# 2gunsu/monocon-pytorch

Measured on AMD Instinct MI355X. Metric: images/sec (384x1280) fwd+bwd, higher is better.
Workload: dtype f32 (f16x2); 1 GPU; train step B=32/GPU 3x384x1280 (configs[2] shape, fp32 values, mode f16x2); global_batch=32, parallelism=dp1, precision_mode=f16x2

## Files before the change

### include/monocon_hip.h

```cpp
#ifndef MONOCON_HIP_H
#define MONOCON_HIP_H

#include <stddef.h>
#include <stdint.h>

#ifdef __cplusplus
extern "C" {
#endif

typedef struct mc_handle mc_handle;

enum { MC_F32 = 0, MC_I64 = 1 };

typedef struct mc_tensor_desc {
    const char *name;
    void *ptr;
    int64_t numel;
    int32_t dtype;
} mc_tensor_desc;

enum {
    MC_PRED_CENTER_HEATMAP = 0, MC_PRED_KPT_HEATMAP, MC_PRED_WH, MC_PRED_OFFSET,
    MC_PRED_KPT_HEATMAP_OFFSET, MC_PRED_CENTER2KPT_OFFSET, MC_PRED_DIM, MC_PRED_DEPTH,
    MC_PRED_ALPHA_CLS, MC_PRED_ALPHA_OFFSET, MC_NUM_PREDS
// ... 32 lines not shown
        *alpha_offset_target, *depth_target, *center2kpt_offset_target, *kpt_heatmap_target,
        *kpt_heatmap_offset_target;
    int64_t *indices, *indices_kpt;
    uint8_t *mask_target;
    float *mask_center2kpt_offset, *mask_kpt_heatmap_offset;
} mc_targets;
int mc_make_targets(mc_handle *h, const mc_labels *labels, int B, int max_objs, int pad_h,
                    int pad_w, int feat_h, int feat_w, const mc_targets *targets, void *stream);
int mc_losses(mc_handle *h, const float *const preds[MC_NUM_PREDS], const mc_targets *targets,
              int B, int max_objs, int feat_h, int feat_w, float *losses, void *stream);
int mc_losses_backward(mc_handle *h, const float *const preds[MC_NUM_PREDS],
                       const mc_targets *targets, int B, int max_objs, int feat_h, int feat_w,
                       const float *grad_losses, float *const dpreds[MC_NUM_PREDS], void *stream);
int mc_losses_backward_pred(mc_handle *h, const float *const preds[MC_NUM_PREDS],
                            const mc_targets *targets, int B, int max_objs, int feat_h, int feat_w,
                            const float *grad_losses, float *const dpreds[MC_NUM_PREDS], void *stream);

int mc_forward_train(mc_handle *h, const float *img, const mc_labels *labels, int B, int H, int W,
                     int max_objs, float *const preds[MC_NUM_PREDS], float *losses, void *stream);
int mc_backward(mc_handle *h, const float *grad_losses, void *stream);
int mc_backward_pred_grads(mc_handle *h, const float *grad_losses, const float *const grad_preds[MC_NUM_PREDS],
                           void *stream);
int mc_backward_image_grad(mc_handle *h, const float *grad_losses, const float *const grad_preds[MC_NUM_PREDS],
                           float *grad_img, void *stream);
int mc_train_generation(mc_handle *h, unsigned long long *generation);
int mc_head_forward_train(mc_handle *h, const float *feat, const mc_labels *labels, int B, int pad_h, int pad_w,
                          int max_objs, float *const preds[MC_NUM_PREDS], float *losses, void *stream);
int mc_head_backward(mc_handle *h, const float *grad_losses, float *grad_feat, void *stream);
int mc_head_backward_pred_grads(mc_handle *h, const float *grad_losses, const float *const grad_preds[MC_NUM_PREDS],
                                float *grad_feat, void *stream);
int mc_train_debug_node(mc_handle *h, int node, int which, float *out_nchw, int dims[4], void *stream);
int mc_infer_debug_node(mc_handle *h, int node, int which, float *out_nchw, int dims[4], void *stream);

int mc_comm_unique_id(mc_handle *h, void *id128);
int mc_comm_init(mc_handle *h, int rank, int world, const void *id128);
int mc_comm_destroy(mc_handle *h);
int mc_comm_set_overlap(mc_handle *h, int on);
int mc_comm_info(mc_handle *h, int *rank, int *world, int *overlap, int *n_collectives, unsigned long long *launches,
                 char *lib_path, int lib_path_len);
int mc_comm_exposed_ms(mc_handle *h, float *ms);
int mc_allreduce_grads(mc_handle *h, void *stream);
int mc_build_train_plan(mc_handle *h, int B, int H, int W);
int mc_tune_export(mc_handle *h, int *buf, int cap, int *n_ints);
int mc_tune_import(mc_handle *h, const int *buf, int n_ints);

int mc_optim_bind(mc_handle *h, int n, float *const params[], float *const grads[],
                  float *const exp_avg[], float *const exp_avg_sq[], const int64_t numel[]);
int mc_clip_adamw_step(mc_handle *h, double lr, double beta1, double beta2, double eps,
                       double weight_decay, double max_norm, int step, float *out_norm, void *stream);

#define MC_OPT_MAX_CLASSES 16
typedef struct mc_optim_class {
    double lr, beta1, beta2, eps, weight_decay;
    int step, amsgrad, maximize;
} mc_optim_class;
int mc_optim_bind_classes(mc_handle *h, int n, float *const params[], float *const grads[],
                          float *const exp_avg[], float *const exp_avg_sq[],
                          float *const max_exp_avg_sq[], const int64_t numel[], const int cls[]);
int mc_clip_adamw_step_classes(mc_handle *h, const mc_optim_class *classes, int ncls, double max_norm,
                               double norm_type, float *out_norm, void *stream);
int mc_clip_bind(mc_handle *h, int n, float *const grads[], const int64_t numel[]);
int mc_clip_grad_norm(mc_handle *h, double max_norm, double norm_type, float *out_norm, void *stream);

int mc_op_conv(mc_handle *h, const float *const src[], const int src_channels[], int nsrc,
               int B, int Hin, int Win, const float *weight_oihw, int Cout, int ksize,
               int stride, const float *scale, const float *bias, const float *residual,
               int relu, float *out, void *stream);
int mc_op_conv_wgrad(mc_handle *h, const float *const src[], const int src_channels[], int nsrc,
                     int B, int Hin, int Win, const float *dy, int Cout, int ksize, int stride,
                     float *dw_oihw, void *stream);
int mc_op_stem(mc_handle *h, const float *img_nchw, int B, int H, int W,
               const float *weight_oihw, const float *scale, const float *bias, float *out,
               void *stream);
int mc_op_stem_dgrad(mc_handle *h, const float *dy_nhwc, const float *weight_oihw, int B, int H, int W,
                     float *dx_nchw, void *stream);
int mc_op_stem_dgrad_fused(mc_handle *h, const float *d_nhwc, const float *y_nhwc, const float *coef,
                           const float *weight_oihw, int B, int H, int W, float *dx_nchw, void *stream);
int mc_op_maxpool2(mc_handle *h, const float *in, int B, int H, int W, int C, float *out,
                   void *stream);
int mc_op_deconv4x4(mc_handle *h, const float *in, int B, int H, int W, int C,
                    const float *weight, float *out, void *stream);
int mc_op_conv_dgrad(mc_handle *h, const float *dy, const float *weight_oihw, int B, int Hin, int Win, int CinTotal,
                     int c_off, int Cs, int Cout, int ksize, int stride, int accumulate, float *dx, void *stream);
int mc_op_nchw_to_nhwc(mc_handle *h, const float *in, int B, int C, int H, int W, float *out,
                       void *stream);
int mc_op_nhwc_to_nchw(mc_handle *h, const float *in, int B, int C, int H, int W, float *out,
                       void *stream);

int mc_preprocess(mc_handle *h, const void *img_hwc, int dtype, int H, int W, const double mean[3],
                  const double std[3], int pad_h, int pad_w, float *out_chw, void *stream);

int mc_preprocess_augmented(mc_handle *h, const unsigned char *frames_hwc, const float *params, int B, int src_h, int src_w,
                            const double mean[3], const double std[3], int pad_h, int pad_w, float *out_bchw, void *stream);

int mc_kitti_format(mc_handle *h, const float *box2d, const float *box3d, const int64_t *cls, const uint8_t *keep_thr,
                    const float *P2, const float *img_hw_scale, int B, int K, float *rows3d, int *n3d, float *rows2d,
                    int *n2d, void *stream);

int mc_nms3d(mc_handle *h, const float *box2d, const float *box3d, const int64_t *cls, const uint8_t *keep_in,
             int B, int K, int mode, float iou_thr, int class_agnostic,
             uint8_t *keep_out, int *suppressed_by, void *stream);

int mc_rotate_iou_eval(mc_handle *h, const float *boxes, const float *query_boxes, long long N, long long K,
                       int criterion, float *iou, void *stream);
int mc_box3d_overlap(mc_handle *h, const double *boxes, const double *query_boxes, long long N, long long K,
                     int criterion, double *overlap, void *stream);

int mc_kitti_image_overlap(const double *boxes, long long N, const double *query_boxes, long long K, int criterion,
                           double *overlap);
int mc_kitti_statistics_part(int mode, const double *overlaps, long long n_frames, const long long *gt_nums,
                             const long long *dt_nums, const long long *dc_nums, const double *gt_datas,
                             const double *dt_datas, const double *dontcares, const long long *ignored_gts,
                             const long long *ignored_dets, int metric, double min_overlap, const double *thresholds,
                             long long n_thresholds, int compute_aos, double *pr, double *scores_out,
                             long long *n_scores);

int mc_query_workspace(mc_handle *h, int B, int H, int W, int mode, size_t *bytes);

int mc_profile_train(mc_handle *h, int iters, double ms[3], double flops[3], double bytes[3], int launches[3],
                     void *stream);
int mc_set_precision(mc_handle *h, int mode);
int mc_set_conv_cfg(mc_handle *h, int cfg);
int mc_bench_conv(mc_handle *h, int B, int Hin, int Win, int nsrc, const int src_channels[],
                  int Cout, int ksize, int stride, int cfg, int iters, float *ms_avg);

int mc_bench_mfma_peak(mc_handle *h, int waves_per_simd, int iters, float *tflops);

size_t mc_workspace_bytes(mc_handle *h);
int mc_forward_cost(mc_handle *h, int B, int H, int W, double flops[2], double bytes[2]);
int mc_profile_forward(mc_handle *h, int iters, float out_ms[3], int out_n[3], void *stream);

#ifdef __cplusplus
}
#endif
#endif
```

### monocon-pytorch_amd/csrc/conv_bf16.hip

```cpp
#include "conv_mfma.h"

namespace mc {

typedef __bf16 bf16x8 __attribute__((ext_vector_type(8)));
typedef __bf16 bf16x4 __attribute__((ext_vector_type(4)));
typedef _Float16 f16x8 __attribute__((ext_vector_type(8)));
typedef _Float16 f16x4 __attribute__((ext_vector_type(4)));

template <int SPL> struct Piece { typedef __bf16 T; typedef bf16x8 V8; typedef bf16x4 V4; };
template <> struct Piece<2> { typedef _Float16 T; typedef f16x8 V8; typedef f16x4 V4; };
__device__ __forceinline__ f32x16 mfma_k16(bf16x8 a, bf16x8 b, f32x16 c) { return __builtin_amdgcn_mfma_f32_32x32x16_bf16(a, b, c, 0, 0, 0); }
__device__ __forceinline__ f32x16 mfma_k16(f16x8 a, f16x8 b, f32x16 c) { return __builtin_amdgcn_mfma_f32_32x32x16_f16(a, b, c, 0, 0, 0); }

template <int KS, int S, int WM, int WN, int WTM, int WTN, int SPL>
struct ConvCfgB16 {
    static constexpr int CK = 32;
    static constexpr int PB = WM * WTM, BNT = WN * WTN * 32, NT = 64 * WM * WN;
    static constexpr int KH = win_h(KS), KW = win_w(KS), PAD = win_pad(KS);
    static constexpr int IH = 3 * S + KH, IW = 7 * S + KW, NPIX = IH * IW;
    static constexpr int ROWB = (CK + 8) * 2;
    static constexpr bool PLANAR = S == 1;
    static constexpr int RS = 24;
    static constexpr int PPB = IH * RS * 16;
    static constexpr int CPL = ((PB + 1) / 2) * PPB + 32;
    static_assert(!PLANAR || (2 * IW <= RS && CK == 32), "two patches per 24-slot row, four 16-byte chunks per pixel");
    static constexpr int PLANE_BYTES = PLANAR ? 4 * CPL : PB * NPIX * ROWB;
    static constexpr int TILE_BYTES = SPL * PLANE_BYTES;
    static constexpr size_t LDS_BYTES = TILE_BYTES + PB * 16;
};

template <int KS, int S, int WM, int WN, int WTM, int WTN, int SPL, bool BM = false, bool LZ = false>
__global__ __launch_bounds__(64 * WM * WN, SPL == 1 ? 3 : 2) void conv_bf16_kernel(const ConvArgs a) {
    static_assert(!LZ || (SPL == 2 && !BM), "lazy sources: forward launches of the fp16-split mode");
    using Cfg = ConvCfgB16<KS, S, WM, WN, WTM, WTN, SPL>;
    typedef typename Piece<SPL>::T pc_t;
    typedef typename Piece<SPL>::V8 pc8;
    typedef typename Piece<SPL>::V4 pc4;
    constexpr int PLANE = Cfg::PLANE_BYTES;
    constexpr int CK = Cfg::CK, PB = Cfg::PB, BNT = Cfg::BNT, NT = Cfg::NT, PAD = Cfg::PAD;
    constexpr int IW = Cfg::IW, NPIX = Cfg::NPIX, ROWB = Cfg::ROWB;
    constexpr bool PLANAR = Cfg::PLANAR;
    constexpr int RS = Cfg::RS, PPB = Cfg::PPB, CPL = Cfg::CPL;
    constexpr int C4 = CK / 4;
    static_assert(NT % C4 == 0, "a thread keeps one channel group across its staging elements");

    extern __shared__ __attribute__((aligned(16))) unsigned char lds_raw[];
    int *pinfo = reinterpret_cast<int *>(lds_raw + Cfg::TILE_BYTES);

    const int tid = threadIdx.x;
    const int lane = tid & 63;
    const int wave = __builtin_amdgcn_readfirstlane(tid >> 6);
    const int wm = wave / WN, wn = wave % WN;
    const int g = lane >> 5, li = lane & 31;

    int img, chunk, n0;
    conv_wg<BNT>(a, img, chunk, n0);

    unsigned am_raw[4] = {0u, 0u, 0u, 0u};
    if constexpr (SPL == 2) {
        const int al = lane < AMAX_SUB ? lane * AMAX_STRIDE : 0;
#pragma unroll
        for (int i = 0; i < 4; ++i) am_raw[i] = a.amax_in[i < a.nsrc ? i : 0][al];
    }

    if (tid < PB) {
        const int pp = chunk * PB + tid;
        const int valid = pp < a.ppi;
        const int py = pp / a.ppr, px = pp % a.ppr;
        pinfo[tid * 4 + 0] = img;
        pinfo[tid * 4 + 1] = py * 4;
        pinfo[tid * 4 + 2] = px * 8;
        pinfo[tid * 4 + 3] = valid;
    }
    __syncthreads();

    float a_scale = 1.f, omul = 1.f;
    auto operand_scales = [&] {
        if constexpr (SPL == 2) {
            unsigned v = am_raw[0];
#pragma unroll
            for (int i = 1; i < 4; ++i) v = am_raw[i] > v ? am_raw[i] : v;
            v = lane < AMAX_SUB ? v : 0u;
#pragma unroll
            for (int o = 8; o > 0; o >>= 1) { const unsigned t = (unsigned)__shfl_xor((int)v, o); v = t > v ? t : v; }
            const int ea = f16_scale_exp((unsigned)__builtin_amdgcn_readfirstlane((int)v));
            const int ew = f16_scale_exp(*a.amax_w);
            a_scale = exp2i(ea);
            omul = exp2i(-ea) * exp2i(-ew);
        }
    };
    constexpr int NACC = SPL >= 2 ? 2 : 1;
    f32x16 acc[WTM][WTN], accm[NACC == 2 ? WTM : 1][NACC == 2 ? WTN : 1];
#pragma unroll
    for (int tm = 0; tm < WTM; ++tm)
#pragma unroll
        for (int tn = 0; tn < WTN; ++tn)
#pragma unroll
            for (int r = 0; r < 16; ++r) {
                acc[tm][tn][r] = 0.f;
                if (NACC == 2) accm[tm][tn][r] = 0.f;
            }

    constexpr int TOTAL = PB * NPIX * C4;
    constexpr int NIT = (TOTAL + NT - 1) / NT;
    const int c4 = tid % C4;
    unsigned char *stage_dst = lds_raw + (tid / C4) * ROWB + c4 * 8;

    int a_off[WTM];
#pragma unroll
    for (int tm = 0; tm < WTM; ++tm) {
        const int p = wm * WTM + tm;
        a_off[tm] = PLANAR ? g * CPL + (p >> 1) * PPB + ((li >> 3) * RS + (li & 7) + IW * (p & 1)) * 16
                           : (p * NPIX + ((li >> 3) * S) * IW + (li & 7) * S) * ROWB + g * 16;
    }

    const int Cin8 = a.Cin >> 3;
    const int w_plane = Cfg::KH * Cfg::KW * a.Cin * a.CoutP * 2;
    const __amdgpu_buffer_rsrc_t r_w = make_rsrc(a.wpk16, (unsigned)(SPL * w_plane));
    const int w_lane = (g * a.CoutP + n0 + wn * WTN * 32 + li) * 16;

    constexpr int KSTEPS = CK / 16, NS = Cfg::KH * Cfg::KW * KSTEPS;
    auto load_b = [&](pc8(&dst)[SPL][WTN], int kc, int s) {
        const int tap = s / KSTEPS, m = s % KSTEPS;
        const int soff = (tap * Cin8 + ((kc + m * 16) >> 3)) * a.CoutP * 16;
#pragma unroll
        for (int q = 0; q < SPL; ++q)
#pragma unroll
            for (int tn = 0; tn < WTN; ++tn)
                dst[q][tn] = __builtin_bit_cast(
                    pc8, __builtin_amdgcn_raw_buffer_load_b128(r_w, w_lane + tn * 32 * 16, soff + q * w_plane, 0));
    };
    auto load_a = [&](pc8(&dst)[SPL][WTM], int s) {
        const int tap = s / KSTEPS, m = s % KSTEPS;
#pragma unroll
        for (int q = 0; q < SPL; ++q)
#pragma unroll
            for (int tm = 0; tm < WTM; ++tm)
                dst[q][tm] = *reinterpret_cast<const pc8 *>(
                    lds_raw + q * PLANE + a_off[tm] +
                    (PLANAR ? 2 * m * CPL + ((tap / Cfg::KW) * RS + (tap % Cfg::KW)) * 16
                            : ((tap / Cfg::KW) * IW + (tap % Cfg::KW)) * ROWB + m * 32));
    };
#ifndef MC_CONV_DB_REGS
#define MC_CONV_DB_REGS 48
#endif
    constexpr int DB_FIT = MC_CONV_DB_REGS / (SPL * WTN * 4);
    constexpr int DB = (WTM * WTN > 2) ? 2 : ((DB_FIT >= 6 && NS % 6 == 0) ? 6 : ((DB_FIT >= 3 && NS % 3 == 0) ? 3 : 2));
    static_assert(NS % DB == 0, "ring slots must line up across K-chunks");
    pc8 bq[DB][SPL][WTN];
#pragma unroll
    for (int j = 0; j < DB - 1; ++j) load_b(bq[j], 0, j);
    const EpiCoef<WTN> coef = conv_epi_coef<WN, WTN, BM>(a, n0, wn, li);

#ifndef MC_CONV_PF
#define MC_CONV_PF 1
#endif
    constexpr bool PF = MC_CONV_PF && NIT <= 8 && WTM * WTN <= 2;
    constexpr int UB = NIT > 8 ? 8 : NIT;
    f32x4 pv[PF ? NIT : 1];
    int voff[NIT], sdst[NIT];
    int si = 0, c0 = 0, kc = 0;
    int Cs = a.src[0].C;
    f32x4 lzA = {0.f, 0.f, 0.f, 0.f}, lzB = lzA;
    bool lz_cur = false, lz_next = false;
    auto lazy_fetch = [&](int s_idx, int cc0) {
        if constexpr (LZ) {
            lz_next = a.src[s_idx].la != nullptr;
            if (lz_next) {
                lzA = reinterpret_cast<const f32x4 *>(a.src[s_idx].la + cc0)[c4];
                lzB = reinterpret_cast<const f32x4 *>(a.src[s_idx].lb + cc0)[c4];
            }
        }
    };
    auto lazy_advance = [&] {
        if constexpr (LZ) {
            lz_cur = lz_next;
            if (lz_cur) {
#pragma unroll
                for (int j = 0; j < 4; ++j) { lzA[j] *= a_scale; lzB[j] *= a_scale; }
            }
        }
    };
    __amdgpu_buffer_rsrc_t r_in = make_rsrc(a.src[0].p + (size_t)img * a.Hin * a.Win * Cs, (unsigned)(a.Hin * a.Win * Cs) * 4u);
    auto lane_offsets = [&](int cs) {
#pragma unroll
        for (int i = 0; i < NIT; ++i) {
            const int e = tid + NT * i;
            const int t = e / C4;
            const int pix = t % NPIX;
            const int p = (t / NPIX) % PB;
            const int iy = pix / IW, ix = pix % IW;
            const int y = pinfo[p * 4 + 1] * S - PAD + iy;
            const int x = pinfo[p * 4 + 2] * S - PAD + ix;
            const bool ok = (e < TOTAL) & (pinfo[p * 4 + 3] != 0) & ((unsigned)y < (unsigned)a.Hin) & ((unsigned)x < (unsigned)a.Win);
            int off = ((y * a.Win + x) * cs + c4 * 4) * 4;
            asm volatile("" : "+v"(off));
            voff[i] = ok ? off : BUF_OOB;
            sdst[i] = PLANAR ? (c4 >> 1) * CPL + (p >> 1) * PPB + (iy * RS + ix + IW * (p & 1)) * 16 + (c4 & 1) * 8
                             : (int)(stage_dst - lds_raw) + i * (NT / C4) * ROWB;
        }
    };
    auto stage_load = [&](__amdgpu_buffer_rsrc_t r, int vo, int so) -> f32x4 { return buf_load4(r, vo, so); };
    auto stage_one = [&](const f32x4 &v, int i, auto lz_c) {
        constexpr bool LZC = decltype(lz_c)::value;
        if (i < NIT && (NT * (i + 1) <= TOTAL || tid + NT * i < TOTAL)) {
            pc4 q[SPL];
            [[maybe_unused]] const float cap = voff[i] != BUF_OOB ? __builtin_inff() : 0.f;
#pragma unroll
            for (int j = 0; j < 4; ++j) {
                float r = SPL == 2 ? (LZC ? lazy_act(v[j], lzA[j], lzB[j], cap) : v[j] * a_scale) : v[j];
#pragma unroll
                for (int pz = 0; pz < SPL; ++pz) {
                    q[pz][j] = (pc_t)r;
                    r -= (float)q[pz][j];
                }
            }
#pragma unroll
            for (int pz = 0; pz < SPL; ++pz) *reinterpret_cast<pc4 *>(lds_raw + sdst[i] + pz * PLANE) = q[pz];
        }
    };
#ifdef MC_PHASE_TIMERS
    unsigned long long tp_stage = 0, tp_bar = 0, tp_mfma = 0, tp_epi = 0;
    const unsigned long long tp_t0 = __builtin_readcyclecounter();
#define TP_NOW() __builtin_readcyclecounter()
#else
#define TP_NOW() 0ull
#endif
    lane_offsets(Cs);
    lazy_fetch(0, 0);
    if (PF) {
#pragma unroll
        for (int i = 0; i < NIT; ++i) pv[i] = stage_load(r_in, voff[i], 0);
    }
    __builtin_amdgcn_sched_barrier(0);
    operand_scales();
// ... 12 lines not shown
                    f32x4 v[UB];
#pragma unroll
                    for (int u = 0; u < UB; ++u)
                        if (i0 + u < NIT) v[u] = stage_load(r_in, voff[i0 + u], c0 * 4);
#pragma unroll
                    for (int u = 0; u < UB; ++u) stage_one(v[u], i0 + u, lz_c);
                }
            }
        };
        if constexpr (LZ) {
            if (lz_cur) stage_chunk(std::true_type{});
            else stage_chunk(std::false_type{});
        } else {
            stage_chunk(std::false_type{});
        }
        [[maybe_unused]] unsigned long long tp_c = TP_NOW();
        __syncthreads();
        [[maybe_unused]] unsigned long long tp_d = TP_NOW();
        int nsi = si, nc0 = c0 + CK;
        if (nc0 >= Cs) { ++nsi; nc0 = 0; }
        const bool more = nsi < a.nsrc;
        if (more && nsi != si) {
            Cs = a.src[nsi].C;
            r_in = make_rsrc(a.src[nsi].p + (size_t)img * a.Hin * a.Win * Cs, (unsigned)(a.Hin * a.Win * Cs) * 4u);
            lane_offsets(Cs);
        }
        if (more) lazy_fetch(nsi, nc0);
        if (PF && more) {
#pragma unroll
            for (int i = 0; i < NIT; ++i) pv[i] = stage_load(r_in, voff[i], nc0 * 4);
        }
        {
            const int kc_next = (kc + CK < a.Cin) ? kc + CK : kc;
            pc8 acur[SPL][WTM];
            load_a(acur, 0);
#pragma unroll
            for (int s = 0; s < NS; ++s) {
                pc8 anext[SPL][WTM];
                if (s + 1 < NS) load_a(anext, s + 1);
                {
                    const int t = s + DB - 1;
                    if (t < NS) load_b(bq[t % DB], kc, t);
                    else load_b(bq[t % DB], kc_next, t - NS);
                }
                __builtin_amdgcn_sched_barrier(0);
                constexpr int NP = SPL == 1 ? 1 : (SPL == 2 ? 3 : 6);
                constexpr int PA[6] = {SPL == 2 ? 1 : 0, SPL == 2 ? 0 : 2, SPL == 2 ? 0 : 1, 0, 1, 0};
                constexpr int PBv[6] = {SPL == 2 ? 0 : 2, SPL == 2 ? 1 : 0, SPL == 2 ? 0 : 1, 1, 0, 0};
#pragma unroll
                for (int pp = 0; pp < NP; ++pp)
#pragma unroll
                    for (int tm = 0; tm < WTM; ++tm)
#pragma unroll
                        for (int tn = 0; tn < WTN; ++tn) {
                            if (NACC == 2 && pp < NP - 1)
                                accm[tm][tn] = mfma_k16(acur[PA[pp]][tm], bq[s % DB][PBv[pp]][tn], accm[tm][tn]);
                            else
                                acc[tm][tn] = mfma_k16(acur[SPL == 1 ? 0 : PA[pp]][tm], bq[s % DB][SPL == 1 ? 0 : PBv[pp]][tn], acc[tm][tn]);
                        }
                if (s + 1 < NS) {
#pragma unroll
                    for (int q = 0; q < SPL; ++q)
#pragma unroll
                        for (int tm = 0; tm < WTM; ++tm) acur[q][tm] = anext[q][tm];
                }
            }
        }
#ifdef MC_PHASE_TIMERS
        { const unsigned long long tp_e = TP_NOW(); tp_bar += (tp_b - tp_a) + (tp_d - tp_c); tp_stage += tp_c - tp_b; tp_mfma += tp_e - tp_d; }
#endif
        if (!more) break;
        si = nsi; c0 = nc0; kc += CK;
    }
    [[maybe_unused]] const unsigned long long tp_f = TP_NOW();

    if (NACC == 2) {
#pragma unroll
        for (int tm = 0; tm < WTM; ++tm)
#pragma unroll
            for (int tn = 0; tn < WTN; ++tn)
#pragma unroll
                for (int r = 0; r < 16; ++r) acc[tm][tn][r] += accm[tm][tn][r];
    }
    conv_epilogue<WM, WN, WTM, WTN, BNT, BM>(a, acc, pinfo, chunk * PB, img, n0, wm, wn, g, li, coef, omul);
#ifdef MC_PHASE_TIMERS
    if (a.phase_prof && lane == 0) {
        __builtin_amdgcn_s_waitcnt(0);
        const unsigned long long tp_g = TP_NOW();
        tp_epi = tp_g - tp_f;
        unsigned long long *o = a.phase_prof + ((size_t)blockIdx.x * (NT / 64) + wave) * 5;
        o[0] = tp_stage; o[1] = tp_bar; o[2] = tp_mfma; o[3] = tp_epi; o[4] = tp_g - tp_t0;
    }
#endif
}

template <int KS, int S, class Sh, int SPL, bool BM = false, bool LZ = false>
static hipError_t launch_b16_one(ConvArgs a, hipStream_t st, ConvArgs *resolved) {
    using Cfg = ConvCfgB16<KS, S, Sh::WM, Sh::WN, Sh::WTM, Sh::WTN, SPL>;
    static_assert(Cfg::PB == Sh::PB && Cfg::BNT == Sh::BNT, "the shape table and the kernel agree on the tile");
    if constexpr (!LZ) {
        if (conv_any_lazy(a)) {
            if constexpr (SPL == 2 && !BM && (KS == 3 || KS == 1)) {
                if (a.bm_y) return hipErrorInvalidValue;
                return launch_b16_one<KS, S, Sh, SPL, false, true>(a, st, resolved);
            } else {
                return hipErrorInvalidValue;
            }
        }
    }
    if constexpr (!BM && S == 1 && (KS == 3 || KS == 1)) {
        if (a.bm_y) return launch_b16_one<KS, S, Sh, SPL, true>(a, st, resolved);
    } else if constexpr (!BM) {
        if (a.bm_y) return hipErrorInvalidValue;
    }
    conv_set_patches(a, Cfg::PB);
    if (a.CoutP % Cfg::BNT) return hipErrorInvalidValue;
    if (resolved) *resolved = a;
    return launch_dyn_lds<conv_bf16_kernel<KS, S, Sh::WM, Sh::WN, Sh::WTM, Sh::WTN, SPL, BM, LZ>>(
        Cfg::LDS_BYTES, dim3((unsigned)(a.B * a.chunks * (a.CoutP / Cfg::BNT))), dim3(Cfg::NT), st, a);
}

bool conv_bf16_ok(const ConvArgs &a, int ks, int stride) {
    if (!a.wpk16) return false;
    if (a.prec == 3) {
        if (!a.amax_w) return false;
        for (int i = 0; i < a.nsrc; ++i)
            if (!a.amax_in[i]) return false;
    }
    for (int i = 0; i < a.nsrc; ++i)
        if (a.src[i].C % 32) return false;
    if (ks == 3) return stride == 1 || stride == 2;
    return stride == 1 && (ks == 1 || ks == 12 || ks == 21 || ks == 22);
}

template <int SPL>
static hipError_t launch_conv_b16_spl(const ConvArgs &a, int ks, int stride, hipStream_t st, ConvArgs *resolved) {
    return with_conv_window(ks, stride, [&](auto win) {
        return with_conv_shape(a.cfg, [&](auto sh) {
            return launch_b16_one<decltype(win)::KS, decltype(win)::S, decltype(sh), SPL>(a, st, resolved);
        });
    });
}

hipError_t launch_conv_bf16(const ConvArgs &a, int ks, int stride, hipStream_t st, ConvArgs *resolved) {
    if (!conv_bf16_ok(a, ks, stride)) return hipErrorInvalidValue;
    if (a.prec == 3) return launch_conv_b16_spl<2>(a, ks, stride, st, resolved);
    return a.prec == 2 ? launch_conv_b16_spl<3>(a, ks, stride, st, resolved) : launch_conv_b16_spl<1>(a, ks, stride, st, resolved);
}

}
```

### monocon-pytorch_amd/csrc/conv_mfma.h

```cpp
#pragma once
#include <hip/hip_runtime.h>
#include <stdint.h>
#include <atomic>
#include <type_traits>
#include <utility>

namespace mc {

typedef float f32x16 __attribute__((ext_vector_type(16)));
typedef float f32x4 __attribute__((ext_vector_type(4)));

struct DynLdsOnce {
    std::atomic<unsigned long long> done{0};
    hipError_t ensure(const void *fn, int bytes) {
        int dev = 0;
        if (hipGetDevice(&dev) != hipSuccess || dev < 0 || dev >= 64) return hipFuncSetAttribute(fn, hipFuncAttributeMaxDynamicSharedMemorySize, bytes);
        if ((done.load(std::memory_order_acquire) >> dev) & 1ull) return hipSuccess;
        const hipError_t e = hipFuncSetAttribute(fn, hipFuncAttributeMaxDynamicSharedMemorySize, bytes);
        if (e == hipSuccess) done.fetch_or(1ull << dev, std::memory_order_release);
        return e;
    }
};

struct ConvSrc {
    const float *p;
    int C;
    const float *la, *lb;
};
__device__ __forceinline__ float lazy_act(float y, float a, float b, float cap) {
    return __builtin_amdgcn_fmed3f(__builtin_fmaf(y, a, b), 0.f, cap);
}

struct ConvArgs {
    ConvSrc src[4];
    int nsrc;
    int B, Hin, Win, Hout, Wout;
    int Cin;
    int Cout, CoutP;
    const float *wpk;
    const float *scale;
    const float *bias;
    const float *res;
    int res_ld;
    float *out;
    int out_ld, out_coff;
    int relu;
    float *stats;
    const float *stat_shift;
    int stats_centred;
    int ppr, ppi, chunks;
    int cfg;
    int o_img, o_row, o_px, r_img, r_row, r_px;
    const void *wpk16;
    int prec;
    const float *bm_y;
    const float *bm_z;
    const unsigned *bm_zbits;
    const float *bm_a, *bm_b;
    int bm_relu;
    const unsigned *amax_in[4];
    const unsigned *amax_w;
    unsigned *amax_out;
    unsigned long long *phase_prof;
};

__host__ __device__ __forceinline__ int f16_scale_exp(unsigned amax_bits) {
    const int E = (int)((amax_bits >> 23) & 0xffu);
    if (E == 0) return 0;
    const int e = 141 - E;
    return e > 126 ? 126 : e;
}
__host__ __device__ __forceinline__ float exp2i(int e) {
    const unsigned u = (unsigned)(127 + e) << 23;
    return __builtin_bit_cast(float, u);
}
constexpr int AMAX_SUB = 16, AMAX_STRIDE = 64, AMAX_WORDS = AMAX_SUB * AMAX_STRIDE;
__device__ __forceinline__ void amax_commit(unsigned *slot, unsigned bits) {
    unsigned *p = slot + (blockIdx.x % AMAX_SUB) * AMAX_STRIDE;
    if (bits < 0x7f800000u && bits > __hip_atomic_load(p, __ATOMIC_RELAXED, __HIP_MEMORY_SCOPE_AGENT)) atomicMax(p, bits);
}
__device__ __forceinline__ void amax_update_block(unsigned *slot, float v) {
    __shared__ unsigned s_amax;
    if (threadIdx.x == 0) s_amax = 0u;
    __syncthreads();
    const unsigned bits = __builtin_bit_cast(unsigned, v);
    if (bits < 0x7f800000u && bits != 0u) atomicMax(&s_amax, bits);
    __syncthreads();
    if (threadIdx.x == 0) amax_commit(slot, s_amax);
}
__device__ __forceinline__ void amax_update_wave(unsigned *slot, float v) {
#pragma unroll
    for (int o = 32; o > 0; o >>= 1) v = fmaxf(v, __shfl_xor(v, o));
    if ((threadIdx.x & 63) == 0) amax_commit(slot, __builtin_bit_cast(unsigned, v));
}
__device__ __forceinline__ unsigned amax_read(const unsigned *slot) {
    const int lane = threadIdx.x & 63;
    unsigned v = lane < AMAX_SUB ? slot[lane * AMAX_STRIDE] : 0u;
#pragma unroll
    for (int o = 8; o > 0; o >>= 1) { const unsigned t = (unsigned)__shfl_xor((int)v, o); v = t > v ? t : v; }
    return (unsigned)__builtin_amdgcn_readfirstlane((int)v);
}

constexpr int win_h(int ks) { return ks >= 10 ? ks / 10 : ks; }
constexpr int win_w(int ks) { return ks >= 10 ? ks % 10 : ks; }
constexpr int win_pad(int ks) { return ks == 3 ? 1 : 0; }

template <int KS, int S, int CK, int WM, int WN, int WTM, int WTN>
struct ConvCfg {
    static constexpr int PB = WM * WTM;
    static constexpr int BNT = WN * WTN * 32;
    static constexpr int NT = 64 * WM * WN;
    static constexpr int KH = win_h(KS), KW = win_w(KS);
    static constexpr int PAD = win_pad(KS);
    static constexpr int IH = 3 * S + KH;
    static constexpr int IW = 7 * S + KW;
    static constexpr int NPIX = IH * IW;
    static constexpr int CKP = CK + 4;
    static constexpr int LDS_FLOATS = PB * NPIX * CKP + PB * 4;
    static constexpr size_t LDS_BYTES = sizeof(float) * LDS_FLOATS;
};

constexpr int BUF_OOB = (int)0x80000000;
typedef int i32x4 __attribute__((ext_vector_type(4)));
__device__ __forceinline__ __amdgpu_buffer_rsrc_t make_rsrc(const void *base, unsigned bytes) {
    return __builtin_amdgcn_make_buffer_rsrc(const_cast<void *>(base), 0, (int)bytes, 0x00020000);
}
__device__ __forceinline__ f32x4 buf_load4(__amdgpu_buffer_rsrc_t r, int voff, int soff) {
    return __builtin_bit_cast(f32x4, __builtin_amdgcn_raw_buffer_load_b128(r, voff, soff, 0));
}
__device__ __forceinline__ float buf_load1(__amdgpu_buffer_rsrc_t r, int voff, int soff) {
    return __builtin_bit_cast(float, __builtin_amdgcn_raw_buffer_load_b32(r, voff, soff, 0));
}
__device__ __forceinline__ void buf_store1(float v, __amdgpu_buffer_rsrc_t r, int voff, int soff) {
    __builtin_amdgcn_raw_buffer_store_b32(__builtin_bit_cast(int, v), r, voff, soff, 0);
}

#ifndef MC_XCD_ORDER
#define MC_XCD_ORDER 1
#endif
__device__ __forceinline__ int xcd_order(int b, int n) {
    if (!MC_XCD_ORDER) return b;
    const int xcd = b & 7, idx = b >> 3, q = n >> 3, r = n & 7;
    return (xcd < r ? xcd * (q + 1) : r * (q + 1) + (xcd - r) * q) + idx;
}

template <int BNT>
__device__ __forceinline__ void conv_wg(const ConvArgs &a, int &img, int &chunk, int &n0) {
// ... 205 lines not shown
struct ConvShapeC {
    static constexpr int WM = CONV_SHAPES[I].WM, WN = CONV_SHAPES[I].WN, WTM = CONV_SHAPES[I].WTM, WTN = CONV_SHAPES[I].WTN;
    static constexpr int PB = CONV_SHAPES[I].PB(), BNT = CONV_SHAPES[I].BNT();
};
template <typename F, int... I>
inline hipError_t with_conv_shape_seq(int id, F &f, std::integer_sequence<int, I...>) {
    hipError_t e = hipErrorInvalidValue;
    (void)((CONV_SHAPES[I].id == id && ((e = f(ConvShapeC<I>{})), true)) || ...);
    return e;
}
template <typename F>
inline hipError_t with_conv_shape(int cfg, F &&f) {
    return with_conv_shape_seq(cfg & CFG_SHAPE_BITS, f, std::make_integer_sequence<int, CONV_NSHAPES>{});
}
template <int KS_, int S_>
struct ConvWin { static constexpr int KS = KS_, S = S_; };
template <typename F>
inline hipError_t with_conv_window(int ks, int stride, F &&f) {
    if (ks == 3 && stride == 1) return f(ConvWin<3, 1>{});
    if (ks == 3 && stride == 2) return f(ConvWin<3, 2>{});
    if (stride != 1) return hipErrorInvalidValue;
    if (ks == 1) return f(ConvWin<1, 1>{});
    if (ks == 12) return f(ConvWin<12, 1>{});
    if (ks == 21) return f(ConvWin<21, 1>{});
    if (ks == 22) return f(ConvWin<22, 1>{});
    return hipErrorInvalidValue;
}

template <auto Kern, typename... Args>
inline hipError_t launch_dyn_lds(size_t lds_bytes, dim3 grid, dim3 block, hipStream_t st, const Args &...args) {
    if (lds_bytes > 160 * 1024) return hipErrorInvalidValue;
    static DynLdsOnce attr_set;
    const hipError_t e = attr_set.ensure(reinterpret_cast<const void *>(Kern), (int)lds_bytes);
    if (e != hipSuccess) return e;
    hipLaunchKernelGGL(Kern, grid, block, lds_bytes, st, args...);
    return hipGetLastError();
}

inline int conv_ntile(int Cout) { return Cout >= 128 ? 128 : (Cout > 32 ? 64 : 32); }
inline int conv_coutp(int Cout) {
    const int t = conv_ntile(Cout);
    return (Cout + t - 1) / t * t;
}
inline int conv_out_dim(int in, int ks, int stride) { return (in + 2 * (ks / 2) - ks) / stride + 1; }
inline int split_pieces(int prec) { return prec == 2 ? 3 : (prec == 3 ? 2 : 1); }
inline int conv_ck(int ks, int stride, const int *src_c, int nsrc) {
    bool all32 = true;
    for (int i = 0; i < nsrc; ++i) all32 = all32 && (src_c[i] % 32 == 0);
    if (ks == 3 && stride == 2) return 16;
    return all32 ? 32 : 16;
}
int conv_pick_cfg(int Cout, int CoutP, int ks, int stride, int B, int Hout, int Wout);
inline int conv_chunks_per_image(int cfg, int Hout, int Wout) {
    if (cfg == CFG_SMALL) return Hout;
    return ((Wout + 7) / 8) * ((Hout + 3) / 4);
}
inline void conv_set_patches(ConvArgs &a, int PB) {
    a.ppr = (a.Wout + 7) / 8;
    a.ppi = a.ppr * ((a.Hout + 3) / 4);
    a.chunks = (a.ppi + PB - 1) / PB;
}
inline bool any_lazy_src(const ConvSrc *src, int nsrc) {
    for (int i = 0; i < nsrc; ++i)
        if (src[i].la) return true;
    return false;
}
inline bool conv_any_lazy(const ConvArgs &a) { return any_lazy_src(a.src, a.nsrc); }
bool conv_small_ok(const ConvArgs &a, int ks, int stride);
bool conv_small_lazy_ok(const ConvArgs &a, int ks, int stride);
bool conv_bf16_ok(const ConvArgs &a, int ks, int stride);
hipError_t launch_conv_bf16(const ConvArgs &a, int ks, int stride, hipStream_t st, ConvArgs *resolved);
hipError_t launch_absmax(const float *x, size_t n, unsigned *slot, hipStream_t st, bool single_word = false);
bool conv_wres_ok(const ConvArgs &a, int ks, int stride);
hipError_t launch_conv_wres(const ConvArgs &a, int ks, int stride, hipStream_t st, ConvArgs *resolved);
hipError_t launch_conv_small(const ConvArgs &a, int stride, hipStream_t st);
bool conv_thin_ok(const ConvArgs &a, int ks, int stride);
hipError_t launch_conv_thin(const ConvArgs &a, hipStream_t st);
bool dgrad_s2_thin_ok(int prec, int ks, int stride, int dyC, int srcC, int CinTotal, int c_off, const unsigned *amax_dy,
                      const unsigned *amax_w, int H, int W);
hipError_t launch_dgrad_s2_thin(const float *dy, int B, int H, int W, int dyC, const float *w_master, int CinTotal, int c_off, float *out,
                                int accumulate, const unsigned *amax_dy, const unsigned *amax_w, hipStream_t st);

hipError_t launch_conv(const ConvArgs &a, int ks, int stride, hipStream_t st, ConvArgs *resolved = nullptr);
bool conv_lazy_capable(const ConvArgs &a, int ks, int stride);

struct ProfLast { int kind; double flops, bytes; };
extern thread_local ProfLast prof_last;

}
```

### monocon-pytorch_amd/csrc/conv_mfma.hip

```cpp
#include <cstdlib>
#include "conv_mfma.h"

namespace mc {

thread_local ProfLast prof_last = {0, 0.0, 0.0};
static ProfLast conv_cost(const ConvArgs &a, int ks) {
    const double px_in = (double)a.B * a.Hin * a.Win, px_out = (double)a.B * a.Hout * a.Wout;
    const double taps = win_h(ks) * win_w(ks);
    const int extra = (a.res ? 1 : 0) + (a.bm_y ? 1 : 0) + ((a.bm_y && a.bm_relu == 1 && !a.bm_zbits) ? 1 : 0);
    return {1, 2.0 * px_out * a.Cout * a.Cin * taps,
            4.0 * (px_in * a.Cin + px_out * a.Cout * (1 + extra) + taps * a.Cin * a.Cout)};
}

template <int KS, int S, int CK, int WM, int WN, int WTM, int WTN, bool BM = false>
__global__ __launch_bounds__(64 * WM * WN, 3) void conv_mfma_kernel(const ConvArgs a) {
    using Cfg = ConvCfg<KS, S, CK, WM, WN, WTM, WTN>;
    constexpr int PB = Cfg::PB, BNT = Cfg::BNT, NT = Cfg::NT, PAD = Cfg::PAD;
    constexpr int IW = Cfg::IW, NPIX = Cfg::NPIX, CKP = Cfg::CKP;
    constexpr int C4 = CK / 4;
    static_assert(NT % C4 == 0, "a thread keeps one channel group across its staging elements");

    extern __shared__ __attribute__((aligned(16))) float lds[];
    int *pinfo = reinterpret_cast<int *>(lds + PB * NPIX * CKP);

// ... 256 lines not shown
#pragma unroll
            for (int s = 0; s < NS; ++s) {
                f32x4 anext[WTM], bnext[WTN];
                if (s + 1 < NS) {
                    load_a(anext, s + 1);
                    load_b(bnext, kc, s + 1);
                } else {
                    load_b(bnext, kc_next, 0);
                }
                __builtin_amdgcn_sched_barrier(0);
#pragma unroll
                for (int j = 0; j < 4; ++j)
#pragma unroll
                    for (int tm = 0; tm < WTM; ++tm)
#pragma unroll
                        for (int tn = 0; tn < WTN; ++tn)
                            acc[tm][tn] = __builtin_amdgcn_mfma_f32_32x32x2f32(
                                acur[tm][j], bcur[tn][j], acc[tm][tn], 0, 0, 0);
                if (s + 1 < NS) {
#pragma unroll
                    for (int tm = 0; tm < WTM; ++tm) acur[tm] = anext[tm];
                }
#pragma unroll
                for (int tn = 0; tn < WTN; ++tn) bcur[tn] = bnext[tn];
            }
            if (ci + 1 < nch) __syncthreads();
        }
        conv_epilogue<WM, WN, WTM, WTN, BNT>(a, acc, pinfo, chunk * PB, img, n0, wm, wn, g, li, coef);
    }
}

template <int KS, int S, int CK, class Sh, bool BM = false>
static hipError_t launch_one(ConvArgs a, hipStream_t st, ConvArgs *resolved) {
    using Cfg = ConvCfg<KS, S, CK, Sh::WM, Sh::WN, Sh::WTM, Sh::WTN>;
    static_assert(Cfg::PB == Sh::PB && Cfg::BNT == Sh::BNT, "the shape table and the kernel agree on the tile");
    if constexpr (!BM && S == 1 && (KS == 3 || KS == 1)) {
        if (a.bm_y) return launch_one<KS, S, CK, Sh, true>(a, st, resolved);
    } else if constexpr (!BM) {
        if (a.bm_y) return hipErrorInvalidValue;
    }
    conv_set_patches(a, Cfg::PB);
    if (a.CoutP % Cfg::BNT) return hipErrorInvalidValue;
    if (resolved) *resolved = a;
    return launch_dyn_lds<conv_mfma_kernel<KS, S, CK, Sh::WM, Sh::WN, Sh::WTM, Sh::WTN, BM>>(
        Cfg::LDS_BYTES, dim3((unsigned)(a.B * a.chunks * (a.CoutP / Cfg::BNT))), dim3(Cfg::NT), st, a);
}

template <int KS, int S, int CK, class Sh>
static hipError_t launch_one_ws(ConvArgs a, hipStream_t st, ConvArgs *resolved) {
    using Cfg = ConvCfgWS<KS, S, CK, Sh::WM, Sh::WN, Sh::WTM, Sh::WTN>;
    static_assert(Cfg::PB == Sh::PB && Cfg::BNT == Sh::BNT, "the shape table and the kernel agree on the tile");
    conv_set_patches(a, Cfg::PB);
    if (a.CoutP % Cfg::BNT) return hipErrorInvalidValue;
    if (resolved) *resolved = a;
    return launch_dyn_lds<conv_mfma_ws_kernel<KS, S, CK, Sh::WM, Sh::WN, Sh::WTM, Sh::WTN>>(
        Cfg::LDS_BYTES, dim3((unsigned)(a.B * a.chunks * (a.CoutP / Cfg::BNT))), dim3(Cfg::NT), st, a);
}

template <int KS, int S, int CK>
static hipError_t launch_shape(const ConvArgs &a, hipStream_t st, ConvArgs *resolved) {
    if (a.cfg & ~(CFG_SHAPE_BITS | CFG_WS)) return hipErrorInvalidValue;
    return with_conv_shape(a.cfg, [&](auto sh) {
        using Sh = decltype(sh);
        if constexpr (KS == 3 || KS == 1)
            if ((a.cfg & CFG_WS) && !a.bm_y) return launch_one_ws<KS, S, CK, Sh>(a, st, resolved);
        return launch_one<KS, S, CK, Sh>(a, st, resolved);
    });
}

int conv_pick_cfg(int Cout, int CoutP, int ks, int stride, int B, int Hout, int Wout) {
    (void)B; (void)Hout; (void)Wout; (void)CoutP;
    const int nt = conv_ntile(Cout);
    if (nt == 128) return ks == 1 ? CFG_64x128 : CFG_128x128;
    if (nt == 64) return (ks == 1 || stride == 2) ? CFG_64x64 : CFG_128x64m;
    return CFG_128x32;
}

bool conv_lazy_capable(const ConvArgs &a, int ks, int stride) {
    if (a.prec != 3 || a.bm_y) return false;
    if (conv_thin_ok(a, ks, stride) || conv_small_lazy_ok(a, ks, stride)) return true;
    return conv_bf16_ok(a, ks, stride) && (ks == 3 || ks == 1);
}

hipError_t launch_conv(const ConvArgs &a_in, int ks, int stride, hipStream_t st, ConvArgs *resolved) {
    ConvArgs a = a_in;
    const bool lazy = conv_any_lazy(a);
    const bool dense_out = a.o_px == 0;
    if (dense_out) { a.o_px = a.out_ld; a.o_row = a.Wout * a.out_ld; a.o_img = a.Hout * a.Wout * a.out_ld; }
    if (a.r_px == 0) { a.r_px = a.res_ld; a.r_row = a.Wout * a.res_ld; a.r_img = a.Hout * a.Wout * a.res_ld; }
    if (a.cfg == CFG_SMALL && !dense_out) return hipErrorInvalidValue;
    int sc[4];
    for (int i = 0; i < a.nsrc; ++i) sc[i] = a.src[i].C;
    const int ck = conv_ck(ks, stride, sc, a.nsrc);
    for (int i = 0; i < a.nsrc; ++i)
        if (sc[i] % ck) return hipErrorInvalidValue;
    if (a.cfg == CFG_SMALL) {
        if (!conv_small_ok(a, ks, stride)) return hipErrorInvalidValue;
        if (lazy && !conv_thin_ok(a, ks, stride) && !conv_small_lazy_ok(a, ks, stride)) return hipErrorInvalidValue;
        conv_set_patches(a, 1);
        a.chunks = a.Hout;
        if (resolved) *resolved = a;
        prof_last = conv_cost(a, ks);
        return launch_conv_small(a, stride, st);
    }
    if (a.cfg == CFG_AUTO) a.cfg = conv_pick_cfg(a.Cout, a.CoutP, ks, stride, a.B, a.Hout, a.Wout);
    prof_last = conv_cost(a, ks);
    if (a.cfg & CFG_WRES) {
        static const bool wres_on = [] { const char *e = std::getenv("MONOCON_HIP_WRES"); return !e || std::atoi(e) != 0; }();
        if (wres_on && conv_wres_ok(a, ks, stride)) return launch_conv_wres(a, ks, stride, st, resolved);
        a.cfg &= ~CFG_WRES;
    }
    if (a.prec >= 1 && conv_bf16_ok(a, ks, stride)) return launch_conv_bf16(a, ks, stride, st, resolved);
    if (lazy) return hipErrorInvalidValue;
    if (ks >= 10) a.cfg &= ~CFG_WS;
    return with_conv_window(ks, stride, [&](auto win) {
        constexpr int KS = decltype(win)::KS, S = decltype(win)::S;
        if constexpr (!(KS == 3 && S == 2))
            if (ck == 32) return launch_shape<KS, S, 32>(a, st, resolved);
        return launch_shape<KS, S, 16>(a, st, resolved);
    });
}

}
```

### monocon-pytorch_amd/csrc/mc_api.hip

```cpp
#include <hip/hip_runtime.h>

#include <algorithm>
#include <cmath>
#include <cstdarg>
#include <cstdio>
#include <cstring>
#include <cstdlib>
#include <map>
#include <memory>
#include <string>
#include <unordered_map>
#include <vector>

#include "../../include/monocon_hip.h"
#include "conv_mfma.h"
#include "kernels.h"

#include <cstdint>
#include "mc_internal.h"

std::string g_create_err;

float *PlanAlloc::alloc(size_t nfloats) {
    const size_t bytes = (nfloats ? nfloats : empty_floats) * sizeof(float);
// ... 196 lines not shown

namespace {
struct Builder {
    mc_handle *h;
    Plan *pl;
    bool ok = true;
    PlanAlloc mem{h, pl->mem, ok, 4, 256};

    Tensor alloc(int B, int H, int W, int C) {
        Tensor t;
        t.B = B; t.H = H; t.W = W; t.C = C;
        t.p = mem.alloc(t.numel());
        t.amax = mem.slot();
        return t;
    }

    void push_conv(Op &op) {
        const ConvArgs &a = op.ca;
        op.kind = OP_CONV;
        const double out_elems = (double)a.B * a.Hout * a.Wout * a.Cout;
        op.flops = 2.0 * out_elems * a.Cin * op.ks * op.ks;
        op.bytes = 4.0 * ((double)a.B * a.Hin * a.Win * a.Cin + out_elems * (a.res ? 2 : 1));
        pl->ops.push_back(op);
    }

    Tensor conv(const ConvLayer &L, const std::vector<const Tensor *> &srcs, const Tensor *res, bool relu) {
        Op op{};
        op.ks = L.ks; op.stride = L.stride;
        ConvArgs &a = op.ca;
        if (!conv_fwd_args(a, L, srcs, h->prec)) { ok = false; h->err = "channel mismatch at " + L.conv; }
        Tensor out = alloc(a.B, a.Hout, a.Wout, L.cout);
        a.amax_out = out.amax;
        a.scale = L.scale; a.bias = L.shift;
        a.res = res ? res->p : nullptr;
        a.res_ld = res ? res->C : 0;
        a.out = out.p; a.out_ld = out.C;
        a.relu = relu ? 1 : 0;
        a.cfg = L.cfg ? L.cfg : (ok ? mc_choose_conv_cfg(h, a, L.ks, L.stride) : CFG_128x32);
        push_conv(op);
        return out;
    }

    Tensor head_conv(const Tensor &feat) {
        const ConvLayer &L = h->head3;
        Tensor hidden = alloc(feat.B, feat.H, feat.W, L.cout);
        Op op{};
        op.ks = L.ks; op.stride = L.stride;
        ConvArgs &a = op.ca;
        pl->head_chunks = mc_head_conv_args(h, mem, feat, hidden.p, a);
        pl->head_stats = a.stats;
        a.amax_out = hidden.amax;
        a.stats_centred = 1;
        if (a.Hout % 4 || a.Wout % 8 || pl->head_chunks != (a.Hout / 4) * (a.Wout / 8)) { ok = false; h->err = "statistics of partial patches at " + L.conv; }
        push_conv(op);
        return hidden;
    }

    Tensor pool(const Tensor &x) {
        Tensor o = alloc(x.B, x.H / 2, x.W / 2, x.C);
        o.amax = x.amax;
        Op op{};
        op.kind = OP_POOL;
        op.in = x.p; op.out = o.p; op.B = x.B; op.H = x.H; op.W = x.W; op.C = x.C;
        op.bytes = 4.0 * ((double)x.numel() + (double)o.numel());
        pl->ops.push_back(op);
        return o;
    }

    Tensor deconv(const DeconvLayer &D, const Tensor &x) {
        Tensor o = alloc(x.B, x.H * 2, x.W * 2, x.C);
        Op op{};
        op.kind = OP_DECONV;
        op.in = x.p; op.out = o.p; op.w = D.wpk; op.B = x.B; op.H = x.H; op.W = x.W; op.C = x.C;
        op.amax = o.amax;
        op.flops = 2.0 * 4.0 * (double)o.numel();
        op.bytes = 4.0 * ((double)x.numel() + (double)o.numel());
        pl->ops.push_back(op);
        return o;
    }
};
}

int mc_choose_conv_cfg(mc_handle *h, const ConvArgs &a_in, int ks, int stride) {
    const bool small_ok = conv_small_ok(a_in, ks, stride);
    if (h->dry_alloc)
        return (small_ok && !(a_in.prec >= 1 && conv_bf16_ok(a_in, ks, stride))) ? (int)CFG_SMALL
                                                                               : conv_pick_cfg(a_in.Cout, a_in.CoutP, ks, stride, a_in.B, a_in.Hout, a_in.Wout);
    if (small_ok && !(a_in.prec >= 1 && conv_bf16_ok(a_in, ks, stride))) return CFG_SMALL;
    if (h->force_cfg) return h->force_cfg;
    int heuristic = small_ok ? (int)CFG_SMALL : conv_pick_cfg(a_in.Cout, a_in.CoutP, ks, stride, a_in.B, a_in.Hout, a_in.Wout);
    if (!h->autotune) return heuristic;
    const bool b16 = a_in.prec >= 1 && conv_bf16_ok(a_in, ks, stride);
    const bool lazy = conv_any_lazy(a_in);
    std::vector<int> key = {a_in.B, a_in.Hin, a_in.Win, ks, stride, a_in.Cout, a_in.CoutP, a_in.nsrc,
                            (a_in.res ? 1 : 0) | (b16 ? 2 * a_in.prec : 0) | (lazy ? 64 : 0)};
    for (int i = 0; i < a_in.nsrc; ++i) key.push_back(a_in.src[i].C);
    auto it = h->tuned.find(key);
    if (it != h->tuned.end()) return it->second;
    static const int cand[] = {CFG_128x128, CFG_128x64, CFG_128x64m, CFG_128x32, CFG_64x128, CFG_64x64,
                               CFG_WS | CFG_128x128, CFG_WS | CFG_128x64m, CFG_WS | CFG_64x128, CFG_WS | CFG_64x64, CFG_SMALL,
                               CFG_WRES | CFG_128x64};
    hipEvent_t e0, e1;
    if (hipEventCreate(&e0) != hipSuccess || hipEventCreate(&e1) != hipSuccess) return heuristic;
    ConvArgs a = a_in;
    a.stats = nullptr;
    int best = heuristic;
    float best_ms = 1e30f;
    for (int c : cand) {
        if (c == CFG_SMALL ? !small_ok : (a.CoutP % conv_shape(c).BNT()) != 0) continue;
        if ((c & CFG_WS) && (ks >= 10 || b16)) continue;
        if ((c & CFG_WRES) && !conv_wres_ok(a, ks, stride)) continue;
        a.cfg = c;
        if (launch_conv(a, ks, stride, nullptr) != hipSuccess) { (void)hipGetLastError(); continue; }
        float t_min = 1e30f;
        for (int rep = 0; rep < 3; ++rep) {
            (void)hipEventRecord(e0, nullptr);
            (void)launch_conv(a, ks, stride, nullptr);
            (void)hipEventRecord(e1, nullptr);
            if (hipEventSynchronize(e1) != hipSuccess) { t_min = 1e30f; break; }
            float ms = 0.f;
            (void)hipEventElapsedTime(&ms, e0, e1);
            t_min = std::min(t_min, ms);
        }
        if (t_min < best_ms) { best_ms = t_min; best = c; }
    }
    (void)hipEventDestroy(e0);
    (void)hipEventDestroy(e1);
    h->tuned[key] = best;
    if (const char *path = std::getenv("MONOCON_HIP_TUNE_CACHE")) {
        if (FILE *f = std::fopen(path, "a")) {
            for (int v : key) std::fprintf(f, "%d ", v);
            std::fprintf(f, ": %d\n", best);
            std::fclose(f);
        }
    }
    return best;
}

static void load_tune_cache(mc_handle *h) {
    const char *path = std::getenv("MONOCON_HIP_TUNE_CACHE");
    if (!path) return;
    FILE *f = std::fopen(path, "r");
    if (!f) return;
    char line[512];
    while (std::fgets(line, sizeof line, f)) {
        std::vector<int> key;
        char *p = line;
        int cfg = -1;
        for (;;) {
            while (*p == ' ') ++p;
            if (*p == ':') { cfg = std::atoi(p + 1); break; }
            if (!*p || *p == '\n') break;
            key.push_back((int)std::strtol(p, &p, 10));
        }
        if (cfg > 0 && key.size() >= 10) h->tuned[key] = cfg;
    }
    std::fclose(f);
}

static Plan *get_plan(mc_handle *h, int B, int H, int W) {
    auto key = std::make_tuple(B, H, W);
    auto it = h->plans.find(key);
    if (it != h->plans.end()) return it->second.get();
    std::unique_ptr<Plan> pl(new Plan());
    pl->B = B; pl->H = H; pl->W = W;
    Builder bd{h, pl.get()};
// ... 941 lines not shown
```

### monocon-pytorch_amd/csrc/mc_train_api.hip

```cpp
#include "mc_internal.h"

#include <algorithm>
#include <cmath>
#include <cstdlib>
#include <cstring>
#include <vector>

static int check_targets(mc_handle *h, const mc_targets *t, const char *who) {
    if (!t) return fail(h, "%s: targets is NULL", who);
    const void *p[] = {t->center_heatmap_target, t->wh_target, t->offset_target, t->dim_target, t->alpha_cls_target,
                       t->alpha_offset_target, t->depth_target, t->center2kpt_offset_target, t->kpt_heatmap_target,
                       t->kpt_heatmap_offset_target, t->indices, t->indices_kpt, t->mask_target,
                       t->mask_center2kpt_offset, t->mask_kpt_heatmap_offset};
    for (size_t i = 0; i < sizeof(p) / sizeof(p[0]); ++i)
        if (!p[i]) return fail(h, "%s: targets field %d is NULL", who, (int)i);
    return 0;
}

extern "C" {

int mc_make_targets(mc_handle *h, const mc_labels *lab, int B, int max_objs, int pad_h, int pad_w, int fh, int fw,
                    const mc_targets *t, void *stream) {
    if (!h) return -1;
    if (!lab || !lab->gt_bboxes || !lab->gt_labels || !lab->gt_bboxes_3d || !lab->depths || !lab->gt_kpts_2d ||
// ... 130 lines not shown
                            int fh, int fw, const float *grad_losses, float *const dpreds[MC_NUM_PREDS], void *stream) {
    return losses_backward_impl(h, preds, t, B, max_objs, fh, fw, grad_losses, dpreds, stream, 1);
}

int mc_op_conv_wgrad(mc_handle *h, const float *const src[], const int src_channels[], int nsrc, int B, int Hin, int Win,
                     const float *dy, int Cout, int ksize, int stride, float *dw_oihw, void *stream) {
    if (!h) return -1;
    if (!src || !src_channels || !dy || !dw_oihw || nsrc < 1 || nsrc > 4) return fail(h, "mc_op_conv_wgrad: bad argument");
    if (!((ksize == 3 && (stride == 1 || stride == 2)) || (ksize == 1 && stride == 1)))
        return fail(h, "mc_op_conv_wgrad: unsupported k=%d stride=%d", ksize, stride);
    if (Cout % 4) return fail(h, "mc_op_conv_wgrad: Cout must be a multiple of 4");
    HIPCHK(h, hipSetDevice(h->device));
    hipStream_t st = static_cast<hipStream_t>(stream);
    Tensor x[4];
    std::vector<const Tensor *> xs;
    for (int i = 0; i < nsrc; ++i) {
        if (!src[i] || src_channels[i] % 16) return fail(h, "mc_op_conv_wgrad: source %d needs C %% 16 == 0", i);
        x[i] = operand_tensor(src[i], B, Hin, Win, src_channels[i]);
        xs.push_back(&x[i]);
    }
    Tensor dyt = operand_tensor(dy, B, mc::conv_out_dim(Hin, ksize, stride), mc::conv_out_dim(Win, ksize, stride), Cout);
    ScratchBuf slots;
    if (h->prec == 3) {
        size_t n[4];
        for (int i = 0; i < nsrc; ++i) n[i] = x[i].numel();
        HIPCHK(h, op_amax_slots(slots, src, n, nsrc, dy, dyt.numel(), false, st));
        for (int i = 0; i < nsrc; ++i) x[i].amax = slots.as<unsigned>() + i * mc::AMAX_WORDS;
        dyt.amax = slots.as<unsigned>() + 4 * mc::AMAX_WORDS;
    }
    mc::WgradArgs a{};
    wgrad_args(a, xs, dyt, Cout, Cout, ksize, stride, h->prec);
    void *part = nullptr;
    HIPCHK(h, hipMalloc(&part, mc::wgrad_partial_floats(a, ksize) * sizeof(float)));
    a.partial = static_cast<float *>(part);
    hipError_t e = mc::launch_wgrad(a, ksize, stride, dw_oihw, st);
    hipError_t e2 = hipStreamSynchronize(st);
    (void)hipFree(part);
    HIPCHK(h, e);
    HIPCHK(h, e2);
    return 0;
}

int mc_op_conv_dgrad(mc_handle *h, const float *dy, const float *weight_oihw, int B, int Hin, int Win, int CinTotal,
                     int c_off, int Cs, int Cout, int ksize, int stride, int accumulate, float *dx, void *stream) {
    if (!h) return -1;
    if (!dy || !weight_oihw || !dx) return fail(h, "mc_op_conv_dgrad: null argument");
    if (!((ksize == 3 && (stride == 1 || stride == 2)) || (ksize == 1 && stride == 1)))
        return fail(h, "mc_op_conv_dgrad: unsupported k=%d stride=%d", ksize, stride);
    if (Cout % 16 || Cs % 4 || c_off < 0 || c_off + Cs > CinTotal) return fail(h, "mc_op_conv_dgrad: bad channel arguments");
    if (stride == 2 && ((Hin | Win) & 1)) return fail(h, "mc_op_conv_dgrad: stride 2 needs even Hin, Win");
    HIPCHK(h, hipSetDevice(h->device));
    hipStream_t st = static_cast<hipStream_t>(stream);
    const int Ho = mc::conv_out_dim(Hin, ksize, stride), Wo = mc::conv_out_dim(Win, ksize, stride);
    const int nclass = stride == 2 ? 4 : 1;
    ScratchBuf slots;
    unsigned *dy_amax = nullptr, *w_amax = nullptr;
    if (h->prec == 3) {
        const size_t ndy = (size_t)B * Ho * Wo * Cout;
        HIPCHK(h, op_amax_slots(slots, &dy, &ndy, 1, weight_oihw, (size_t)Cout * CinTotal * ksize * ksize, true, st));
        dy_amax = slots.as<unsigned>();
        w_amax = dy_amax + 4 * mc::AMAX_WORDS;
    }
    ScratchBuf panel[4], panel16[4];
    mc::PackBatch pack;
    for (int c = 0; c < nclass; ++c) {
        const int cls = stride == 2 ? c : -1;
        const size_t pn = mc::dgrad_panel_elems(ksize, cls, Cout, Cs);
        HIPCHK(h, panel[c].alloc(pn * 4));
        HIPCHK(h, hipMemsetAsync(panel[c].p, 0, pn * 4, st));
        if (mc::panel_has_pieces(h->prec, Cout)) {
            const size_t bytes16 = pn * 2 * mc::split_pieces(h->prec);
            HIPCHK(h, panel16[c].alloc(bytes16));
            HIPCHK(h, hipMemsetAsync(panel16[c].p, 0, bytes16, st));
        }
        pack.add(mc::pack_job_dgrad(weight_oihw, Cout, CinTotal, ksize, c_off, Cs, Cout, cls, panel[c].as<float>(), panel16[c].p,
                                    h->prec, w_amax));
    }
    hipError_t e = pack.launch(st);
    for (int c = 0; c < nclass && e == hipSuccess; ++c) {
        mc::ConvArgs d;
        const int kk = mc::dgrad_conv_args(d, pack.jobs[c], h->prec, dy, dy_amax, B, Ho, Wo, Cout, dx, Hin, Win, accumulate != 0);
        d.cfg = h->force_cfg;
        e = mc::launch_conv(d, kk, 1, st);
    }
    hipError_t e2 = hipStreamSynchronize(st);
    HIPCHK(h, e);
    HIPCHK(h, e2);
    return 0;
}

static int upload_opt_table(mc_handle *h, const std::vector<mc::OptTensor> &tab, const int64_t numel[], mc::OptTensor **dtab,
                            mc::OptChunk **dchunks, int *nchunks) {
    std::vector<mc::OptChunk> chunks;
    const int CH = 1 << 16;
    for (int i = 0; i < (int)tab.size(); ++i)
        for (int64_t b = 0; b < numel[i]; b += CH)
            chunks.push_back(mc::OptChunk{i, (int)b, (int)std::min<int64_t>(CH, numel[i] - b)});
    if (*dtab) (void)hipFree(*dtab);
    if (*dchunks) (void)hipFree(*dchunks);
    *dtab = nullptr; *dchunks = nullptr; *nchunks = 0;
    void *q = nullptr;
    HIPCHK(h, hipMalloc(&q, tab.size() * sizeof(mc::OptTensor)));
    *dtab = static_cast<mc::OptTensor *>(q);
    HIPCHK(h, hipMalloc(&q, chunks.size() * sizeof(mc::OptChunk)));
    *dchunks = static_cast<mc::OptChunk *>(q);
    HIPCHK(h, hipMemcpy(*dtab, tab.data(), tab.size() * sizeof(mc::OptTensor), hipMemcpyHostToDevice));
    HIPCHK(h, hipMemcpy(*dchunks, chunks.data(), chunks.size() * sizeof(mc::OptChunk), hipMemcpyHostToDevice));
    *nchunks = (int)chunks.size();
    if (!h->opt_ws) {
        HIPCHK(h, hipMalloc(&q, (mc::opt_partial_floats() + 8) * sizeof(float)));
        h->opt_ws = static_cast<float *>(q);
    }
    return 0;
}

static int optim_bind(mc_handle *h, const char *who, int n, float *const params[], float *const grads[], float *const exp_avg[],
                      float *const exp_avg_sq[], float *const max_exp_avg_sq[], const int64_t numel[], const int cls[]) {
    if (!h) return -1;
    if (n < 1 || !params || !grads || !exp_avg || !exp_avg_sq || !numel) return fail(h, "%s: bad argument", who);
    HIPCHK(h, hipSetDevice(h->device));
    std::vector<mc::OptTensor> tab(n);
    int max_cls = 0;
    unsigned novmax = 0;
    for (int i = 0; i < n; ++i) {
        if (!params[i] || !grads[i] || !exp_avg[i] || !exp_avg_sq[i] || numel[i] < 1)
            return fail(h, "%s: tensor %d has a null pointer / empty size", who, i);
        if (numel[i] > INT32_MAX) return fail(h, "%s: tensor %d has more than 2^31-1 elements", who, i);
        const int c = cls ? cls[i] : 0;
        if (c < 0 || c >= MC_OPT_MAX_CLASSES)
            return fail(h, "%s: tensor %d has class index %d, outside [0, %d)", who, i, c, MC_OPT_MAX_CLASSES);
        float *vmax = max_exp_avg_sq ? max_exp_avg_sq[i] : nullptr;
        tab[i] = mc::OptTensor{params[i], grads[i], exp_avg[i], exp_avg_sq[i], vmax, c};
        max_cls = std::max(max_cls, c);
        if (!vmax) novmax |= 1u << c;
    }
    h->opt_ntensors = 0;
    if (upload_opt_table(h, tab, numel, &h->opt_tab, &h->opt_chunks, &h->opt_nchunks)) return -1;
    h->opt_ntensors = n;
    h->opt_max_cls = max_cls;
    h->opt_novmax = novmax;
    return 0;
}

int mc_optim_bind(mc_handle *h, int n, float *const params[], float *const grads[], float *const exp_avg[],
                  float *const exp_avg_sq[], const int64_t numel[]) {
    return optim_bind(h, "mc_optim_bind", n, params, grads, exp_avg, exp_avg_sq, nullptr, numel, nullptr);
}

int mc_optim_bind_classes(mc_handle *h, int n, float *const params[], float *const grads[], float *const exp_avg[],
                          float *const exp_avg_sq[], float *const max_exp_avg_sq[], const int64_t numel[], const int cls[]) {
    if (h && !cls) return fail(h, "mc_optim_bind_classes: bad argument");
    return optim_bind(h, "mc_optim_bind_classes", n, params, grads, exp_avg, exp_avg_sq, max_exp_avg_sq, numel, cls);
}

static void fold_hyper(mc::AdamHyper &hp, double lr, double beta1, double beta2, double eps, double weight_decay, int step) {
    const double bc1 = 1.0 - std::pow(beta1, (double)step), bc2 = 1.0 - std::pow(beta2, (double)step);
    hp.decay = (float)(1.0 - lr * weight_decay);
    hp.beta1 = (float)beta1; hp.one_minus_beta1 = (float)(1.0 - beta1);
    hp.beta2 = (float)beta2; hp.one_minus_beta2 = (float)(1.0 - beta2);
    hp.sqrt_bc2 = (float)std::sqrt(bc2);
    hp.eps = (float)eps;
    hp.step_size = (float)(lr / bc1);
}

int mc_clip_adamw_step(mc_handle *h, double lr, double beta1, double beta2, double eps, double weight_decay,
                       double max_norm, int step, float *out_norm, void *stream) {
// ... 82 lines not shown
```

### monocon-pytorch_amd/csrc/mc_train_plan.hip

```cpp
#include <atomic>
#include <deque>
#include <functional>

#include "mc_internal.h"

using namespace mc;

namespace {

using Fn = std::function<int(mc_handle *, hipStream_t)>;

struct PlanSwitches {
    long long lazy_z;
    long long lazy_min;
    long long lazy_feat;
    long long zbits;
    long long grad_pool;
    long long grad_pool_cool;
    long long head_dx_fuse;
    long long head_zskip;
    long long dgrad_s2_thin;
    long long stem_fuse;
    long long bm_epilogue;
    long long wres_bwd;
    long long dual_stream;
    int side_sync_lo = 0, side_sync_hi = 0;
    bool plan_debug = false;
};
const struct { const char *name; long long PlanSwitches::*field; long long def; } SWITCH_TABLE[] = {
    {"MONOCON_HIP_LAZY_Z", &PlanSwitches::lazy_z, 3},
    {"MONOCON_HIP_LAZY_MIN", &PlanSwitches::lazy_min, 900000},
    {"MONOCON_HIP_LAZY_FEAT", &PlanSwitches::lazy_feat, 0},
    {"MONOCON_HIP_ZBITS", &PlanSwitches::zbits, 1},
    {"MONOCON_HIP_GRAD_POOL", &PlanSwitches::grad_pool, 1},
    {"MONOCON_HIP_GRAD_POOL_COOL", &PlanSwitches::grad_pool_cool, 2},
    {"MONOCON_HIP_HEAD_DX_FUSE", &PlanSwitches::head_dx_fuse, 1},
    {"MONOCON_HIP_HEAD_ZSKIP", &PlanSwitches::head_zskip, 1},
    {"MONOCON_HIP_DGRAD_S2_THIN", &PlanSwitches::dgrad_s2_thin, 1},
    {"MONOCON_HIP_STEM_FUSE", &PlanSwitches::stem_fuse, 1},
    {"MONOCON_HIP_BM_EPILOGUE", &PlanSwitches::bm_epilogue, 1},
    {"MONOCON_HIP_WRES_BWD", &PlanSwitches::wres_bwd, 0},
    {"MONOCON_HIP_DUAL_STREAM", &PlanSwitches::dual_stream, 1},
};
PlanSwitches read_switches() {
    PlanSwitches sw{};
    std::string changed;
    for (const auto &d : SWITCH_TABLE) {
        const char *e = std::getenv(d.name);
        sw.*d.field = e ? std::atoll(e) : d.def;
        if (sw.*d.field != d.def) changed += std::string(" ") + d.name + "=" + std::to_string(sw.*d.field);
    }
    if (const char *e = std::getenv("MONOCON_HIP_SIDE_SYNC")) {
        if (std::sscanf(e, "%d:%d", &sw.side_sync_lo, &sw.side_sync_hi) != 2) sw.side_sync_lo = sw.side_sync_hi = 0;
        if (sw.side_sync_lo < sw.side_sync_hi) changed += std::string(" MONOCON_HIP_SIDE_SYNC=") + e;
    }
    sw.plan_debug = std::getenv("MONOCON_HIP_PLAN_DEBUG") != nullptr;
    if (sw.plan_debug && !changed.empty()) fprintf(stderr, "[plan] switches off their defaults:%s\n", changed.c_str());
    return sw;
}

struct PoolBwdArgs {
    const float *x, *dout, *la, *lb;
    float *dx, *stats;
    int B, H, W, C, acc;
};

struct LastWriter {
    enum Kind { NONE, DGRAD_CONV, POOL_BWD, DECONV_BWD } kind = NONE;
    union {
        ConvArgs *conv;
        PoolBwdArgs *pool;
        float **deconv_stats;
    };
    LastWriter() : conv(nullptr) {}
    LastWriter(ConvArgs *c) : kind(c ? DGRAD_CONV : NONE), conv(c) {}
    LastWriter(PoolBwdArgs *p) : kind(p ? POOL_BWD : NONE), pool(p) {}
    LastWriter(float **s) : kind(s ? DECONV_BWD : NONE), deconv_stats(s) {}
};

struct TNode {
    Tensor t;
    float *g = nullptr;
    bool ginit = false, needs_grad = true;
    LastWriter last;
};

enum RecKind { REC_STEM, REC_CONV, REC_POOL, REC_DECONV, REC_HEAD };
struct Rec {
    RecKind kind;
    ConvLayer *L = nullptr;
    DeconvLayer *D = nullptr;
    std::vector<int> srcs;
    int res = -1, z = -1, in = -1;
    bool relu = true, dead = false;
    Tensor y;
    float *mean = nullptr, *rstd = nullptr;
    float *ca = nullptr, *cb = nullptr;
    unsigned *zbits = nullptr;
    std::string bn;
};

enum BwdStream { ON_MAIN, ON_SIDE };
struct BwdStep {
    Fn fn;
    BwdStream stream = ON_MAIN;
    int wait = -1;
    int bucket = -1;
    bool feat_dgrad = false;
    bool img_dgrad = false;
    hipEvent_t ready = nullptr;
    hipEvent_t fin = nullptr;
};

}

struct TrainState {
    int B = 0, H = 0, W = 0;
    unsigned long long bind_gen = 0;
    PlanSwitches sw{};
    PlanMem mem;
    std::vector<TNode> nodes;
    std::vector<Rec> recs;
    std::vector<Fn> fwd;
    std::vector<BwdStep> bwd;
    std::deque<ConvArgs> dgrads;
    std::deque<PoolBwdArgs> pool_bwds;
    std::deque<float *> deconv_stats;
    hipStream_t side = nullptr;
    hipEvent_t side_done = nullptr;
    bool dual = true;
    unsigned *img_amax = nullptr;
    mc::PackBatch pack_batch;
    std::vector<Fn> pack_fns;
    const float *img = nullptr;
    mc_labels labels{};
    float *preds[10] = {nullptr};
    float *losses = nullptr;
    const float *grad_losses = nullptr;
    const float *grad_preds[10] = {nullptr};
    int pad_h = 0, pad_w = 0, max_objs = 30;
    bool head_only = false;
    const float *feat_ext = nullptr;
    float *gfeat_ext = nullptr;
    bool skip_feat_dgrad = false;
    float *gimg_ext = nullptr;
    mc_targets targets{};
    float *dpred[10] = {nullptr};
    bool ok = true;
};

static std::atomic<unsigned long long> g_train_generation{0};

static void train_free(TrainState *t) {
    if (!t) return;
    for (const BwdStep &s : t->bwd) {
        if (s.ready) (void)hipEventDestroy(s.ready);
        if (s.fin) (void)hipEventDestroy(s.fin);
    }
// ... 248 lines not shown
        ts->nodes[o].t.amax = t.amax;
        const float *ip = tx.p, *la = tx.la, *lb = tx.lb;
        float *op = ts->nodes[o].t.p;
        const int B = t.B, H = t.H, W = t.W, C = t.C;
        ts->fwd.push_back([=](mc_handle *hh, hipStream_t st) {
            HIPCHK(hh, launch_maxpool2(ip, B, H, W, C, op, st, la, lb));
            return 0;
        });
        Rec r;
        r.kind = REC_POOL; r.in = x; r.z = o;
        ts->recs.push_back(r);
        return o;
    }

    int deconv(DeconvLayer &D, int x) {
        if (ts->nodes[x].t.la && !ts->nodes[x].t.lrelu) materialise(x);
        const Tensor t = ts->nodes[x].t;
        const int o = node(t.B, t.H * 2, t.W * 2, t.C, true);
        const float *ip = t.p, *w = D.wpk, *la = t.la, *lb = t.lb;
        float *op = ts->nodes[o].t.p;
        unsigned *omax = ts->nodes[o].t.amax;
        const int B = t.B, H = t.H, W = t.W, C = t.C;
        ts->fwd.push_back([=](mc_handle *hh, hipStream_t st) {
            HIPCHK(hh, launch_deconv4(ip, B, H, W, C, w, op, st, omax, la, lb));
            return 0;
        });
        Rec r;
        r.kind = REC_DECONV; r.in = x; r.z = o; r.D = &D;
        ts->recs.push_back(r);
        return o;
    }

    const PackJobDesc &pack_job(const float *w, int Cout, int CinTotal, int k, int c_off, int Cs, int CoutPad, int cls) {
        const size_t pn = dgrad_panel_elems(k, cls, CoutPad, Cs);
        float *dst = alloc(pn);
        void *dst16 = panel_has_pieces(h->prec, CoutPad) ? alloc((3 * pn + 1) / 2) : nullptr;
        ts->pack_batch.add(pack_job_dgrad(w, Cout, CinTotal, k, c_off, Cs, CoutPad, cls, dst, dst16, h->prec, w_slot(w)));
        return ts->pack_batch.jobs.back();
    }

    void emit_dgrad(const float *w_master, const Tensor &dy, int Cout_fwd, int CinTotal, int ks, int stride, int c_off, int srcnode,
                    int CoutPad) {
        TNode &sn = ts->nodes[srcnode];
        if (!sn.needs_grad) return;
        g_acquire(srcnode);
        auto dgrad_conv = [&](int cls, ConvArgs &d) {
            const PackJobDesc &p = pack_job(w_master, Cout_fwd, CinTotal, ks, c_off, sn.t.C, CoutPad, cls);
            return dgrad_conv_args(d, p, h->prec, dy.p, dy.amax, dy.B, dy.H, dy.W, dy.C, sn.g, sn.t.H, sn.t.W, sn.ginit);
        };
        if (stride == 2 && ks == 3) {
            if (2 * dy.H != sn.t.H || 2 * dy.W != sn.t.W) { ts->ok = false; h->err = "train plan: stride-2 dgrad shape mismatch"; }
            if (sw.dgrad_s2_thin && ts->ok && dgrad_s2_thin_ok(h->prec, ks, stride, dy.C, sn.t.C, CinTotal, c_off, dy.amax, w_slot(w_master), dy.H, dy.W)) {
                const float *dyp = dy.p;
                float *gp = sn.g;
                const int B = dy.B, Hd = dy.H, Wd = dy.W, Cd = dy.C, acc = sn.ginit ? 1 : 0;
                const unsigned *dmax = dy.amax, *wmax = w_slot(w_master);
                push_bwd([=](mc_handle *hh, hipStream_t st) {
                    HIPCHK(hh, launch_dgrad_s2_thin(dyp, B, Hd, Wd, Cd, w_master, CinTotal, c_off, gp, acc, dmax, wmax, st));
                    return 0;
                });
                wrote(srcnode);
                return;
            }
            for (int cls = 0; cls < 4; ++cls) {
                ConvArgs d;
                const int kk = dgrad_conv(cls, d);
                d.cfg = ts->ok ? mc_choose_conv_cfg(h, d, kk, 1) : CFG_128x32;
                push_bwd([=](mc_handle *hh, hipStream_t st) { HIPCHK(hh, launch_conv(d, kk, 1, st)); return 0; });
            }
            wrote(srcnode);
            return;
        }
        ConvArgs d;
        dgrad_conv(-1, d);
        if (dy.H != sn.t.H || dy.W != sn.t.W) { ts->ok = false; h->err = "train plan: dgrad shape mismatch"; }
        d.cfg = ts->ok ? mc_choose_conv_cfg(h, d, ks, 1) : CFG_128x32;
        if (sw.wres_bwd < 2) d.cfg &= ~CFG_WRES;
        ts->dgrads.push_back(d);
        ConvArgs *dp = &ts->dgrads.back();
        push_bwd([=](mc_handle *hh, hipStream_t st) { HIPCHK(hh, launch_conv(*dp, ks, 1, st)); return 0; });
        wrote(srcnode, (d.cfg == CFG_SMALL && !conv_thin_ok(d, ks, 1)) ? nullptr : dp);
    }

    int emit_wgrad(const std::vector<int> &srcs, const Tensor &dy, int dy_ld, int Cout, int ks, int stride, float *dw) {
        WgradArgs a{};
        const std::vector<const Tensor *> xs = conv_sources(srcs);
        wgrad_args(a, xs, dy, dy_ld, Cout, ks, stride, h->prec);
        if (wgrad_any_lazy(a) && !wgrad_lazy_capable(a, ks, stride)) {
            for (int s_ : srcs) materialise(s_);
            wgrad_args(a, xs, dy, dy_ld, Cout, ks, stride, h->prec);
        }
        a.partial = alloc(wgrad_partial_floats(a, ks));
        return push_bwd([=](mc_handle *hh, hipStream_t st) { HIPCHK(hh, launch_wgrad(a, ks, stride, dw, st)); return 0; }, ON_SIDE);
    }

    struct BnBwd { Tensor dy; float *coef; bool affine_skipped; };
    BnBwd bn_backward(const Rec &r, const std::string &bn, bool caller_forms_dy = false) {
        TNode &zn = ts->nodes[r.z];
        Tensor dy = r.y;
        dy.p = zn.g;
        dy.amax = slot();
        unsigned *dymax = dy.amax;
        const int B = r.y.B, C = r.y.C, rows = r.y.H * r.y.W;
        const float *yp = r.y.p, *gz = zn.g, *zp = zn.t.p, *gamma = P(bn + ".weight", C), *mean = r.mean, *rstd = r.rstd;
        float *dg = G(bn + ".weight", C), *db = G(bn + ".bias", C), *dyp = dy.p;
        float *coef = alloc((size_t)C * 4);
        const int relu = r.relu ? ((r.res < 0 && r.ca && r.cb) ? 2 : 1) : 0;
        const float *fa = r.ca, *fb = r.cb;
        float *gres = nullptr;
        int gmode = 0;
        if (r.res >= 0 && ts->nodes[r.res].needs_grad) {
            gres = g_acquire(r.res);
            gmode = ts->nodes[r.res].ginit ? 2 : 1;
            wrote(r.res);
        }
        const double n = (double)B * rows;
        auto step = [&](float *partial, int nbp, int cstride, bool reduce, bool affine) {
            double *fold = fold_scratch(nbp, C);
            const int arelu = reduce ? relu : 0;
            const float *aa = reduce ? fa : nullptr, *ab = reduce ? fb : nullptr;
            push_bwd([=](mc_handle *hh, hipStream_t st) {
                if (reduce) HIPCHK(hh, launch_chan_reduce(yp, gz, zp, nullptr, B, rows, C, 1, relu, partial, C, st, fa, fb));
                HIPCHK(hh, launch_bn_bwd_finalize(partial, nbp, cstride, n, C, gamma, mean, rstd, dg, db, coef, st, fold));
                if (affine)
                    HIPCHK(hh, launch_affine_bwd(gz, zp, yp, coef, B, (size_t)rows, C, 0, arelu, dyp, gres, gmode, st, aa, ab, nullptr,
                                                 nullptr, dymax));
                return 0;
            });
            return BnBwd{dy, coef, !affine};
        };
        const LastWriter last = zn.last;
        ConvArgs *lc = last.kind == LastWriter::DGRAD_CONV ? last.conv : nullptr;
        if (sw.bm_epilogue == 0 || (sw.bm_epilogue > 1 && r.y.H * r.y.W > sw.bm_epilogue)) lc = nullptr;
        if (sw.plan_debug)
            fprintf(stderr, "[plan] bn_backward %-40s %4d ch %4dx%-4d relu %d res %d last-writer-conv %d\n", bn.c_str(), C, r.y.H,
                    r.y.W, relu, r.res >= 0, lc != nullptr);
        if (lc && lc->out == zn.g && lc->Cout == C && lc->out_ld == C && lc->Hout == r.y.H && lc->Wout == r.y.W && !lc->stats) {
            const int ppi = conv_chunks_per_image(lc->cfg, r.y.H, r.y.W), nbp = B * ppi, cstride = lc->CoutP;
            float *partial = alloc((size_t)nbp * cstride * 2);
            lc->stats = partial;
            lc->bm_y = yp; lc->bm_z = zp; lc->bm_a = fa; lc->bm_b = fb; lc->bm_relu = relu;
            lc->bm_zbits = relu == 1 ? r.zbits : nullptr;
            if (sw.wres_bwd >= 1 && !(lc->cfg & (CFG_SMALL | CFG_WS)) && conv_wres_ok(*lc, 3, 1)) lc->cfg |= CFG_WRES;
            if (sw.plan_debug)
                fprintf(stderr, "[plan]   twin of %-36s cfg %3d  K %4d  Cout %3d  %dx%d  res %d  nsrc %d srcC %d wres %d\n", bn.c_str(), lc->cfg,
                        lc->Cin, lc->Cout, lc->Hout, lc->Wout, lc->res != nullptr, lc->nsrc, lc->src[0].C, (lc->cfg & CFG_WRES) != 0);
            const bool skip_affine = caller_forms_dy && !gres;
            if (skip_affine) lc->amax_out = dymax;
            return step(partial, nbp, cstride, false, !skip_affine);
        }
        PoolBwdArgs *pl = last.kind == LastWriter::POOL_BWD ? last.pool : nullptr;
        if (pl && relu == 2 && pl->la == fa && pl->lb == fb && pl->x == yp && pl->acc && pl->dx == zn.g && pl->C == C &&
            pl->H * pl->W == rows && !pl->stats && !caller_forms_dy && C % 4 == 0 && 256 % (C / 4) == 0) {
            const int nbp = maxpool2_bwd_blocks(B, pl->H, pl->W, C);
            float *partial = alloc((size_t)nbp * C * 2);
            pl->stats = partial;
            if (sw.plan_debug)
                fprintf(stderr, "[plan]   statistics of %-36s left by the max-pool backward (%d partial rows)\n", bn.c_str(), nbp);
            return step(partial, nbp, C, false, true);
        }
        float **ds = last.kind == LastWriter::DECONV_BWD ? last.deconv_stats : nullptr;
        if (ds && relu == 2 && zn.t.la == fa && zn.t.lb == fb && !*ds && !caller_forms_dy && !gres) {
            const int nbp = B * r.y.H;
            float *partial = alloc((size_t)nbp * C * 2);
            *ds = partial;
            if (sw.plan_debug)
                fprintf(stderr, "[plan]   statistics of %-36s left by the deconv backward (%d partial rows)\n", bn.c_str(), nbp);
            return step(partial, nbp, C, false, true);
        }
        const int nb = chan_reduce_blocks(B, rows);
        return step(alloc((size_t)nb * C * 2), nb, C, true, true);
    }

    static constexpr int CP = NUM_HEADS * HEAD_CH, LD = 80;
    Tensor xh;
    AttnTrainArgs at{};
    AttnGradPtrs gp{};
    float *w3dense = nullptr;
    size_t raw_numel = 0;

    void heads_forward(int feat) {
        xh.B = B; xh.H = fh; xh.W = fw; xh.C = CP; xh.p = alloc(xh.numel());
        Tensor raw; raw.B = B; raw.H = fh; raw.W = fw; raw.C = LD; raw.p = alloc(raw.numel());
        raw_numel = raw.numel();
        for (int hd = 0; hd < NUM_HEADS; ++hd) {
            const std::string an = mc_head_keys(hd).attn;
            const int A = NUM_AFFINE, AC = NUM_AFFINE * HEAD_CH;
            at.rm[hd] = P(an + ".running_mean", HEAD_CH); at.rv[hd] = P(an + ".running_var", HEAD_CH);
            at.nbt[hd] = NBT(an + ".num_batches_tracked");
            at.att_w[hd] = P(an + ".attn_weights.attention.0.weight", AC);
            at.att_g[hd] = P(an + ".attn_weights.attention.1.weight", A);
            at.att_b[hd] = P(an + ".attn_weights.attention.1.bias", A);
            at.att_rm[hd] = P(an + ".attn_weights.attention.1.running_mean", A);
            at.att_rv[hd] = P(an + ".attn_weights.attention.1.running_var", A);
            at.att_nbt[hd] = NBT(an + ".attn_weights.attention.1.num_batches_tracked");
            at.weight_[hd] = P(an + ".weight_", AC); at.bias_[hd] = P(an + ".bias_", AC);
            gp.d_weight_[hd] = G(an + ".weight_", AC); gp.d_bias_[hd] = G(an + ".bias_", AC);
            gp.d_att_w[hd] = G(an + ".attn_weights.attention.0.weight", AC);
            gp.d_att_g[hd] = G(an + ".attn_weights.attention.1.weight", A);
            gp.d_att_b[hd] = G(an + ".attn_weights.attention.1.bias", A);
        }
        ConvArgs c3{};
        at.chunks = mc_head_conv_args(h, mem, ts->nodes[feat].t, xh.p, c3);
        if (conv_any_lazy(c3) && (!ts->nodes[feat].t.lrelu || !conv_lazy_capable(c3, 3, 1))) {
            materialise(feat);
            conv_fwd_args(c3, h->head3, {&ts->nodes[feat].t}, h->prec);
        }
        at.stat_ld = h->head3.coutp;
        at.stats = c3.stats; at.B = B; at.HW = HW;
        at.stats64 = reinterpret_cast<double *>(alloc((size_t)B * at.stat_ld * 4));
        at.sv_inst = alloc((size_t)B * CP * 3); at.mu_r = alloc((size_t)CP * 2); at.bn10 = alloc(NUM_HEADS * NUM_AFFINE * 2);
        at.that = alloc((size_t)B * NUM_HEADS * NUM_AFFINE); at.yatt = alloc((size_t)B * NUM_HEADS * NUM_AFFINE);
        at.gamma_p = alloc((size_t)B * CP); at.scale = alloc((size_t)B * CP); at.shift = alloc((size_t)B * CP);
        w3dense = alloc((size_t)CP * 64 * 9);
        HeadApplyArgs ha{};
        ha.hidden = xh.p; ha.scale = at.scale; ha.shift = at.shift; ha.w = h->head_w1t; ha.b = h->head_b1;
        ha.B = B; ha.HW = HW; ha.z_out = nullptr;
        for (int i = 0; i < 10; ++i) ha.pred_c[i] = PRED_CH[i];
        ts->fwd.push_back([=](mc_handle *hh, hipStream_t st) { HIPCHK(hh, launch_conv(c3, 3, 1, st)); return 0; });
        ts->fwd.push_back([=, ts = ts, at = at](mc_handle *hh, hipStream_t st) {
            HIPCHK(hh, launch_attn_train_fwd(at, st));
            HeadApplyArgs a2 = ha;
            for (int i = 0; i < 10; ++i) a2.pred[i] = ts->preds[i];
            HIPCHK(hh, launch_head_apply(a2, st));
            return 0;
        });
    }

    void targets_and_losses() {
        mc_targets &T = ts->targets;
        const size_t R = (size_t)B * ts->max_objs;
// ... 63 lines not shown
        for (int hd = 0; hd < NUM_HEADS; ++hd)
            for (const HeadOutLayer &o : mc_head_keys(hd).out) seg(o.layer, o.row0, o.rows);
        const float *xp = xh.p, *w1 = h->head_w1, *zsc = at.scale, *zsh = at.shift;
        push_bwd([=, B = B, HW = HW](mc_handle *hh, hipStream_t st) {
            HIPCHK(hh, launch_head_bwd(draw, LD, nullptr, xp, w1, B, HW, nbr, dx_fuse ? nullptr : dh, dw1p, partial, st, zsc, zsh, nz_bwd));
            HIPCHK(hh, launch_splitk_reduce(dw1p, nbr, 1, NUM_OUT_ROWS, HEAD_CH, dw1, st));
            HIPCHK(hh, launch_copy_batch(segcb, st));
            return 0;
        });
        float *db3 = alloc(CP), *dw3 = alloc((size_t)CP * 64 * 9);
        float *cs3 = alloc((size_t)std::max(affine_bwd_blocks(B, (size_t)HW, CP), nbr) * CP * 2);
        Tensor dxT = xh; dxT.p = dx; dxT.amax = slot();
        unsigned *dxmax = dxT.amax;
        push_bwd([=, at = at, gp = gp, B = B, HW = HW](mc_handle *hh, hipStream_t st) {
            HIPCHK(hh, launch_attn_train_bwd(at, partial, rb_per_img, gp, coef, st));
            if (dx_fuse)
                HIPCHK(hh, launch_head_dx(draw, LD, xp, w1, coef, B, HW, nbr, dx, cs3, db3, dxmax, st, zsc, zsh, nz_dx));
            else
                HIPCHK(hh, launch_affine_bwd(dh, nullptr, xp, coef, B, (size_t)HW, CP, 1, 0, dx, nullptr, 0, st, nullptr, nullptr, cs3, db3,
                                             dxmax));
            return 0;
        });
        emit_wgrad({feat}, dxT, CP, CP, 3, 1, dw3);
        CopyBatch g3cb;
        for (int hd = 0; hd < NUM_HEADS; ++hd) {
            const std::string layer = mc_head_keys(hd).conv3;
            if (!g3cb.add(dw3 + (size_t)hd * 64 * 64 * 9, G(layer + ".weight", 9 * HEAD_CH * HEAD_CH), (size_t)64 * 64 * 9) ||
                !g3cb.add(db3 + hd * 64, G(layer + ".bias", HEAD_CH), 64))
                ts->ok = false;
        }
        push_bwd([=](mc_handle *hh, hipStream_t st) { HIPCHK(hh, launch_copy_batch(g3cb, st)); return 0; }, ON_SIDE);
        CopyBatch w3cb;
        for (int hd = 0; hd < NUM_HEADS; ++hd)
            if (!w3cb.add(P(mc_head_keys(hd).conv3 + ".weight", 9 * HEAD_CH * HEAD_CH), w3dense + (size_t)hd * 64 * 64 * 9,
                          (size_t)64 * 64 * 9))
                ts->ok = false;
        ts->pack_fns.push_back([=](mc_handle *hh, hipStream_t st) { HIPCHK(hh, launch_copy_batch(w3cb, st)); return 0; });
        if (h->prec == 3) h->w_amax_of[w3dense] = h->head3.w_amax;
        emit_dgrad(w3dense, dxT, CP, 64, 3, 1, 0, feat, CP);
        if (ts->head_only) ts->bwd.back().feat_dgrad = true;
    }

    void pool_backward(const Rec &r) {
        TNode &in = ts->nodes[r.in];
        const TNode &o = ts->nodes[r.z];
        if (!o.ginit || !in.needs_grad) return;
        float *gi = g_acquire(r.in);
        PoolBwdArgs pa{in.t.p, o.g, in.t.la, in.t.lb, gi, nullptr, in.t.B, in.t.H, in.t.W, in.t.C, in.ginit ? 1 : 0};
        ts->pool_bwds.push_back(pa);
        PoolBwdArgs *pp = &ts->pool_bwds.back();
        push_bwd([=](mc_handle *hh, hipStream_t st) {
            HIPCHK(hh, launch_maxpool2_bwd(pp->x, pp->dout, pp->B, pp->H, pp->W, pp->C, pp->dx, pp->acc, st, pp->la, pp->lb, pp->stats));
            return 0;
        });
        wrote(r.in, pp);
        g_release(r.z, -1);
    }

    void deconv_backward(const Rec &r) {
        TNode &in = ts->nodes[r.in];
        const TNode &o = ts->nodes[r.z];
        if (!o.ginit) return;
        if (in.ginit) { ts->ok = false; h->err = "train plan: deconv input has more than one consumer"; }
        const float *xp = in.t.p, *go = o.g, *wp = r.D->wpk, *xla = in.t.la, *xlb = in.t.lb;
        float *gi = g_acquire(r.in), *dw = G(r.D->name + ".weight", (int64_t)r.D->C * 16);
        const int Bq = in.t.B, Hq = in.t.H, Wq = in.t.W, Cq = in.t.C;
        float *part = alloc(deconv4_bwd_w_partial_floats(Bq, Hq, Cq));
        ts->deconv_stats.push_back(nullptr);
        float **dstats = &ts->deconv_stats.back();
        push_bwd([=](mc_handle *hh, hipStream_t st) {
            HIPCHK(hh, launch_deconv4_bwd_w(xp, go, Bq, Hq, Wq, Cq, part, dw, st, xla, xlb, wp, gi, *dstats));
            return 0;
        });
        wrote(r.in, (xla && xlb) ? dstats : nullptr);
        g_release(r.z, -1);
    }

    void conv_backward(const Rec &r) {
        if (r.dead || !ts->nodes[r.z].ginit) return;
        const Tensor dy = bn_backward(r, r.bn).dy;
        const int64_t wn = (int64_t)r.L->cout * r.L->cin * r.L->ks * r.L->ks;
        const int wgrad = emit_wgrad(r.srcs, dy, r.L->cout, r.L->cout, r.L->ks, r.L->stride, G(r.L->conv + ".weight", wn));
        const float *wm = P(r.L->conv + ".weight", wn);
        int c_off = 0;
        for (int s : r.srcs) {
            emit_dgrad(wm, dy, r.L->cout, r.L->cin, r.L->ks, r.L->stride, c_off, s, r.L->cout);
            c_off += ts->nodes[s].t.C;
        }
        g_release(r.z, wgrad);
    }

    void stem_backward(const Rec &r) {
        if (!ts->nodes[r.z].ginit) return;
        const bool want_fused = sw.stem_fuse && h->prec == 3 && ts->img_amax && r.y.amax && W % 4 == 0 && W >= 16;
        const BnBwd bb = bn_backward(r, r.bn, want_fused);
        const bool fused = bb.affine_skipped;
        float *part = alloc((size_t)stem_wgrad_blocks(B, H, W) * 147 * 16), *dw = G("backbone.base_layer.0.weight", 16 * 147);
        const float *dyp = bb.dy.p, *yfp = fused ? r.y.p : nullptr, *cfp = fused ? bb.coef : nullptr;
        const unsigned *imax = ts->img_amax, *dymax = bb.dy.amax, *yfmax = fused ? r.y.amax : nullptr;
        const int wgrad = push_bwd([=, ts = ts, B = B, H = H, W = W](mc_handle *hh, hipStream_t st) {
            HIPCHK(hh, launch_stem_wgrad(ts->img, dyp, B, H, W, part, dw, st, imax, imax ? dymax : nullptr, yfp, cfp, yfmax));
            return 0;
        }, ON_SIDE);
        const float *wm = P("backbone.base_layer.0.weight", 16 * 147);
        const int dgrad = push_bwd([=, ts = ts, B = B, H = H, W = W](mc_handle *hh, hipStream_t st) {
            if (ts->gimg_ext) HIPCHK(hh, launch_stem_dgrad(dyp, wm, B, H, W, ts->gimg_ext, st, yfp, cfp));
            ts->gimg_ext = nullptr;
            return 0;
        });
        ts->bwd[dgrad].img_dgrad = true;
        ts->bwd[dgrad].bucket = -1;
        g_release(r.z, wgrad);
    }

    void feat_grad_out(int feat) {
        const float *gp = ts->nodes[feat].g;
        push_bwd([=, ts = ts, B = B, fh = fh, fw = fw](mc_handle *hh, hipStream_t st) {
            if (ts->gfeat_ext) HIPCHK(hh, launch_nhwc_to_nchw(gp, B, 64, fh, fw, ts->gfeat_ext, st));
            ts->gfeat_ext = nullptr;
            return 0;
        });
    }
};

}

static TrainState *build_train(mc_handle *h, int B, int H, int W, bool head_only = false) {
    std::unique_ptr<TrainState, void (*)(TrainState *)> tsp(new TrainState(), train_free);
    TrainState *ts = tsp.get();
    ts->B = B; ts->H = H; ts->W = W; ts->bind_gen = h->bind_gen; ts->head_only = head_only;
    ts->sw = read_switches();
    TB b{h, ts};
    b.zero_amax_slots();
    int feat;
    if (head_only) {
        feat = b.external_feat();
    } else {
        b.stem();
        for (const NetStep &s : h->net.steps) {
            const int o = s.kind == STEP_CONV ? b.conv_bn(s) : s.kind == STEP_POOL ? b.pool(s.srcs[0]) : b.deconv(h->deconvs[s.name], s.srcs[0]);
            if (o != s.out) { ts->ok = false; h->err = "train plan: node order differs from the network graph"; }
        }
        feat = h->net.feat;
    }
    b.heads_forward(feat);
    b.targets_and_losses();
    b.cur_bucket = 0;
    b.heads_backward(feat);
    for (int ri = (int)ts->recs.size() - 1; ri >= 0; --ri) {
        const Rec r = ts->recs[ri];
        b.cur_bucket = mc_grad_bucket_of(r.kind == REC_DECONV ? r.D->name : (r.kind == REC_POOL ? std::string("backbone.") : r.bn));
        if (r.kind == REC_POOL) b.pool_backward(r);
        else if (r.kind == REC_DECONV) b.deconv_backward(r);
        else if (r.kind == REC_CONV) b.conv_backward(r);
        else if (r.kind == REC_STEM) b.stem_backward(r);
    }
    if (head_only) b.feat_grad_out(feat);
    {
        bool seen[MC_NUM_GRAD_BUCKETS] = {};
        for (auto s = ts->bwd.rbegin(); s != ts->bwd.rend(); ++s) {
            if (s->bucket < 0) continue;
            if (seen[s->bucket]) s->bucket = -1;
            else seen[s->bucket] = true;
        }
    }
    if (!ts->ok) return nullptr;
    if (ts->sw.plan_debug)
        fprintf(stderr, "[plan] lazy activations: %d never stored, %d stored after all (lazy mask %d), %.2f GB\n", b.n_lazy - b.n_materialised,
                b.n_materialised, (int)ts->sw.lazy_z, ts->mem.bytes * 1e-9);
    if (h->dry_alloc) return tsp.release();
// ... 291 lines not shown
```

### monocon-pytorch_amd/csrc/pack_batch.hip

```cpp
#include "kernels.h"
#include "train.h"
#include "conv_mfma.h"
#include <type_traits>

namespace mc {

__device__ __forceinline__ void store_pieces_b(float r, unsigned short *dst, size_t plane, int nsplit) {
    if (nsplit == 2) {
        const _Float16 hi = (_Float16)r;
        const _Float16 lo = (_Float16)(r - (float)hi);
        dst[0] = __builtin_bit_cast(unsigned short, hi);
        dst[plane] = __builtin_bit_cast(unsigned short, lo);
    } else {
        for (int q = 0; q < nsplit; ++q) {
            const __bf16 piece = (__bf16)r;
            dst[q * plane] = __builtin_bit_cast(unsigned short, piece);
            r -= (float)piece;
        }
    }
}

__global__ __launch_bounds__(256) void weight_amax_batch_kernel(const PackJobDesc *__restrict__ tab, int njobs) {
    int lo = 0, hi = njobs - 1;
    while (lo < hi) {
// ... 67 lines not shown
                typedef unsigned short u8v __attribute__((ext_vector_type(8)));
                float r[8];
#pragma unroll
                for (int q = 0; q < 8; ++q) r[q] = v[q] * wscale;
                for (int pz = 0; pz < j.nsplit; ++pz) {
                    u8v o;
#pragma unroll
                    for (int q = 0; q < 8; ++q) {
                        const __bf16 piece = (__bf16)r[q];
                        o[q] = __builtin_bit_cast(unsigned short, piece);
                        r[q] -= (float)piece;
                    }
                    *reinterpret_cast<u8v *>(d16 + pz * plane + i16) = o;
                }
            }
        }
    };
    if (j.kind == 0) {
        const size_t total = (size_t)j.Cout * j.Cin * kk;
        const size_t plane = (size_t)kk * j.CinTotal * j.CoutP;
        if (j.Cin % 8 == 0 && j.c_off % 8 == 0 && (kk == 9 || kk == 1) && (reinterpret_cast<uintptr_t>(j.w) & 15) == 0) {
            const int items = j.Cout * (j.Cin >> 3);
            auto run = [&](auto kkc) {
                constexpr int KK = decltype(kkc)::value;
                for (int it = lb * 256 + threadIdx.x; it < items; it += j.nblocks * 256) {
                    const int n = it % j.Cout, c8 = it / j.Cout;
                    const int cc = c8 * 8 + j.c_off, nn = n + j.n_off;
                    const float *src = j.w + ((size_t)n * j.Cin + c8 * 8) * KK;
                    float buf[8 * KK];
#pragma unroll
                    for (int q = 0; q < 2 * KK; ++q) {
                        const float4 t = reinterpret_cast<const float4 *>(src)[q];
                        buf[4 * q] = t.x; buf[4 * q + 1] = t.y; buf[4 * q + 2] = t.z; buf[4 * q + 3] = t.w;
                    }
#pragma unroll
                    for (int tap = 0; tap < KK; ++tap) {
                        float v[8];
#pragma unroll
                        for (int q = 0; q < 8; ++q) v[q] = buf[q * KK + tap];
                        const size_t i32a = (((size_t)tap * (j.CinTotal >> 2) + (cc >> 2)) * j.CoutP + nn) * 4;
                        put8(v, i32a, i32a + (size_t)j.CoutP * 4, (((size_t)tap * (j.CinTotal >> 3) + (cc >> 3)) * j.CoutP + nn) * 8, plane);
                    }
                }
            };
            if (kk == 9) run(std::integral_constant<int, 9>{}); else run(std::integral_constant<int, 1>{});
            return;
        }
        for (size_t e = (size_t)lb * 256 + threadIdx.x; e < total; e += (size_t)j.nblocks * 256) {
            const int tap = e % kk;
            const int c = (e / kk) % j.Cin;
            const int n = e / ((size_t)kk * j.Cin);
            const int cc = c + j.c_off, nn = n + j.n_off;
            float r = j.w[e];
            if (j.dst32) j.dst32[(((size_t)tap * (j.CinTotal >> 2) + (cc >> 2)) * j.CoutP + nn) * 4 + (cc & 3)] = r;
            if (d16)
                store_pieces_b(r * wscale, d16 + (((size_t)tap * (j.CinTotal >> 3) + (cc >> 3)) * j.CoutP + nn) * 8 + (cc & 7), plane,
                               j.nsplit);
        }
    } else {
        const int Cs = j.Cin, cls = j.cls, py = cls >> 1, px = cls & 1;
        const size_t total = (size_t)j.Cout * Cs * kk;
        const size_t plane = (size_t)(cls < 0 ? kk : (1 + py) * (1 + px)) * j.CoutP * j.CsP;
        if (j.Cout % 8 == 0 && (kk == 9 || kk == 1)) {
            const int items = Cs * (j.Cout >> 3);
            auto run = [&](auto kc) {
                constexpr int K = decltype(kc)::value, KK = K * K;
                for (int it = lb * 256 + threadIdx.x; it < items; it += j.nblocks * 256) {
                    const int cl = it % Cs, n8 = it / Cs;
                    const float *src = j.w + ((size_t)(n8 * 8) * j.CinTotal + j.c_off + cl) * KK;
#pragma unroll
                    for (int tap = 0; tap < KK; ++tap) {
                        const int r = tap / K, sx = tap % K;
                        int tapd;
                        if (cls < 0) {
                            tapd = (K - 1 - r) * K + (K - 1 - sx);
                        } else {
                            if ((py == 0) != (r == 1) || (px == 0) != (sx == 1)) continue;
                            const int dr = py ? (2 - r) / 2 : 0, ds = px ? (2 - sx) / 2 : 0;
                            tapd = dr * (1 + px) + ds;
                        }
                        float v[8];
#pragma unroll
                        for (int q = 0; q < 8; ++q) v[q] = src[(size_t)q * j.CinTotal * KK + tap];
                        const size_t i32a = (((size_t)tapd * (j.CoutP >> 2) + n8 * 2) * j.CsP + cl) * 4;
                        put8(v, i32a, i32a + (size_t)j.CsP * 4, (((size_t)tapd * (j.CoutP >> 3) + n8) * j.CsP + cl) * 8, plane);
                    }
                }
            };
            if (k == 3) run(std::integral_constant<int, 3>{}); else run(std::integral_constant<int, 1>{});
            return;
        }
        for (size_t e = (size_t)lb * 256 + threadIdx.x; e < total; e += (size_t)j.nblocks * 256) {
            const int tap = e % kk;
            const int cl = (e / kk) % Cs;
            const int n = e / ((size_t)kk * Cs);
            const int r = tap / k, s = tap % k;
            int tapd;
            if (cls < 0) {
                tapd = (k - 1 - r) * k + (k - 1 - s);
            } else {
                if ((py == 0) != (r == 1) || (px == 0) != (s == 1)) continue;
                const int dr = py ? (2 - r) / 2 : 0, ds = px ? (2 - s) / 2 : 0;
                tapd = dr * (1 + px) + ds;
            }
            float rem = j.w[(((size_t)n * j.CinTotal + j.c_off + cl) * k + r) * k + s];
            if (j.dst32) j.dst32[(((size_t)tapd * (j.CoutP >> 2) + (n >> 2)) * j.CsP + cl) * 4 + (n & 3)] = rem;
            if (d16)
                store_pieces_b(rem * wscale, d16 + (((size_t)tapd * (j.CoutP >> 3) + (n >> 3)) * j.CsP + cl) * 8 + (n & 7), plane,
                               j.nsplit);
        }
    }
}

void PackBatch::clear() {
    jobs.clear();
    total_blocks = 0;
    uploaded = false;
}
void PackBatch::add(PackJobDesc j) {
    const size_t total = (size_t)j.Cout * j.Cin * j.k * j.k;
    size_t nb = (total + 1023) / 1024;
    if (nb < 1) nb = 1;
    if (nb > 256) nb = 256;
    j.nblocks = (int)nb;
    j.block_begin = total_blocks;
    total_blocks += (int)nb;
    jobs.push_back(j);
    uploaded = false;
}
hipError_t PackBatch::launch(hipStream_t st, bool with_amax) {
    if (jobs.empty()) return hipSuccess;
    for (const PackJobDesc &j : jobs)
        if (j.nsplit == 2 && j.dst16 && !j.amax) return hipErrorInvalidValue;
    if (!uploaded) {
        if (dev) (void)hipFree(dev);
        dev = nullptr;
        hipError_t e = hipMalloc(reinterpret_cast<void **>(&dev), jobs.size() * sizeof(PackJobDesc));
        if (e != hipSuccess) return e;
        e = hipMemcpy(dev, jobs.data(), jobs.size() * sizeof(PackJobDesc), hipMemcpyHostToDevice);
        if (e != hipSuccess) return e;
        uploaded = true;
    }
    if (with_amax)
        hipLaunchKernelGGL(weight_amax_batch_kernel, dim3((unsigned)total_blocks), dim3(256), 0, st, dev, (int)jobs.size());
    hipLaunchKernelGGL(pack_batch_kernel, dim3((unsigned)total_blocks), dim3(256), 0, st, dev, (int)jobs.size());
    return hipGetLastError();
}
PackBatch::~PackBatch() {
    if (dev) (void)hipFree(dev);
}

__global__ void fold_bn_batch_kernel(const FoldJobDesc *__restrict__ tab) {
    const FoldJobDesc j = tab[blockIdx.y];
    const int c = blockIdx.x * blockDim.x + threadIdx.x;
    if (c >= j.C) return;
    const float inv = 1.0f / sqrtf(j.rv[c] + j.eps);
    const float s = (j.g ? j.g[c] : 1.f) * inv;
    j.scale[c] = s;
    j.shift[c] = (j.b ? j.b[c] : 0.f) - j.rm[c] * s;
}
void FoldBatch::clear() {
    jobs.clear();
    uploaded = false;
    maxC = 0;
}
void FoldBatch::add(const FoldJobDesc &j) {
    jobs.push_back(j);
    if (j.C > maxC) maxC = j.C;
    uploaded = false;
}
hipError_t FoldBatch::launch(hipStream_t st) {
    if (jobs.empty()) return hipSuccess;
    if (!uploaded) {
        if (dev) (void)hipFree(dev);
        dev = nullptr;
        hipError_t e = hipMalloc(reinterpret_cast<void **>(&dev), jobs.size() * sizeof(FoldJobDesc));
        if (e != hipSuccess) return e;
        e = hipMemcpy(dev, jobs.data(), jobs.size() * sizeof(FoldJobDesc), hipMemcpyHostToDevice);
        if (e != hipSuccess) return e;
        uploaded = true;
    }
    hipLaunchKernelGGL(fold_bn_batch_kernel, dim3((unsigned)((maxC + 63) / 64), (unsigned)jobs.size()), dim3(64), 0, st, dev);
    return hipGetLastError();
}
FoldBatch::~FoldBatch() {
    if (dev) (void)hipFree(dev);
}

}
```

### monocon-pytorch_amd/csrc/train.h

```cpp
#pragma once
#include <hip/hip_runtime.h>
#include <stdint.h>
#include <cstdlib>
#include <vector>

#include "conv_mfma.h"

namespace mc {

struct TargetArgs {
    const float *gt_bboxes, *gt_labels, *gt_bboxes_3d, *depths, *gt_kpts_2d, *gt_kpts_valid, *mask;
    int B, max_objs, num_kpt, num_classes, fh, fw;
    float h_ratio, w_ratio;
    float *center_heatmap, *kpt_heatmap;
    float *wh, *offset, *dim, *alpha_cls, *alpha_offset, *depth, *c2k, *kho;
    long long *indices, *indices_kpt;
    uint8_t *mask_target;
    float *mask_c2k, *mask_kho;
};
hipError_t launch_make_targets(const TargetArgs &a, hipStream_t st);

hipError_t launch_focal(const float *p, const float *t, size_t n, float *partial, float *loss_out, float *aux,
                        hipStream_t st);
hipError_t launch_focal_grad(const float *p, const float *t, size_t n, const float *aux, const float *gscale, int gidx,
                             float *dlogit, hipStream_t st, int wrt_pred = 0);
int focal_partial_floats();

struct GatherLossArgs {
    const float *pred[10];
    float *dpred[10];
    const long long *indices, *indices_kpt;
    const uint8_t *mask_target;
    const float *wh, *offset, *dim, *alpha_cls, *alpha_offset, *depth, *c2k, *kho, *mask_c2k, *mask_kho;
    int B, max_objs, HW;
    float *losses;
    float *aux;
    const float *gscale;
    int wrt_pred;
    double *partial;
    int nwg;
};
size_t gathered_loss_ws_doubles();
hipError_t launch_gathered_losses(const GatherLossArgs &a, int mode, hipStream_t st);

struct PackJobDesc {
    const float *w;
    float *dst32;
    void *dst16;
    int kind;
    int Cout, Cin, k;
    int CinTotal;
    int CoutP;
    int n_off, c_off;
    int CsP, cls, nsplit;
    int block_begin, nblocks;
    unsigned *amax;
};
inline bool panel_has_pieces(int prec, int K) { return prec >= 1 && K % 8 == 0; }
inline int dgrad_taps(int k, int cls) { return cls < 0 ? k * k : (1 + (cls >> 1)) * (1 + (cls & 1)); }
inline size_t fwd_panel_elems(int k, int CinPanel, int CoutP) { return (size_t)k * k * CinPanel * CoutP; }
inline size_t dgrad_panel_elems(int k, int cls, int CoutPad, int Cs) { return (size_t)dgrad_taps(k, cls) * CoutPad * conv_coutp(Cs); }
inline PackJobDesc pack_job_fwd(const float *w, int Cout, int Cin, int k, float *dst32, void *dst16, int CinPanel, int CoutP,
                                int n_off, int prec, unsigned *amax) {
    PackJobDesc j{};
    j.w = w; j.dst32 = dst32; j.dst16 = panel_has_pieces(prec, CinPanel) ? dst16 : nullptr;
    j.kind = 0; j.Cout = Cout; j.Cin = Cin; j.k = k; j.CinTotal = CinPanel; j.CoutP = CoutP; j.n_off = n_off;
    j.cls = -1; j.nsplit = split_pieces(prec); j.amax = amax;
    return j;
}
inline PackJobDesc pack_job_dgrad(const float *w, int Cout, int CinTotal, int k, int c_off, int Cs, int CoutPad, int cls,
                                  float *dst32, void *dst16, int prec, unsigned *amax) {
    PackJobDesc j{};
    j.w = w; j.dst32 = dst32; j.dst16 = panel_has_pieces(prec, CoutPad) ? dst16 : nullptr;
    j.kind = 1; j.Cout = Cout; j.Cin = Cs; j.k = k; j.CinTotal = CinTotal; j.CoutP = CoutPad; j.c_off = c_off;
    j.CsP = conv_coutp(Cs); j.cls = cls; j.nsplit = split_pieces(prec); j.amax = amax;
    return j;
}
inline int dgrad_conv_args(ConvArgs &d, const PackJobDesc &p, int prec, const float *dy, const unsigned *dy_amax, int B, int Hd,
                           int Wd, int Cd, float *g, int Hs, int Ws, bool accumulate) {
    const int ld = p.Cin, py = p.cls >> 1, px = p.cls & 1;
    d = ConvArgs{};
    d.nsrc = 1; d.src[0].p = dy; d.src[0].C = Cd;
    d.B = B; d.Hin = Hd; d.Win = Wd; d.Hout = Hd; d.Wout = Wd;
    d.Cin = Cd; d.Cout = ld; d.CoutP = p.CsP; d.wpk = p.dst32;
    d.wpk16 = p.dst16; d.prec = p.dst16 ? prec : 0;
    d.amax_in[0] = dy_amax; d.amax_w = p.amax;
    d.out = g; d.out_ld = ld;
    if (p.cls >= 0) {
        d.out = g + ((size_t)py * Ws + px) * ld;
        d.o_px = 2 * ld; d.o_row = 2 * Ws * ld; d.o_img = Hs * Ws * ld;
    }
    if (accumulate) { d.res = d.out; d.res_ld = ld; d.r_px = d.o_px; d.r_row = d.o_row; d.r_img = d.o_img; }
    if (p.cls < 0) return p.k;
    const int code = (1 + py) * 10 + (1 + px);
    return code == 11 ? 1 : code;
}
struct PackBatch {
    std::vector<PackJobDesc> jobs;
    PackJobDesc *dev = nullptr;
    int total_blocks = 0;
    bool uploaded = false;
    void clear();
    void add(PackJobDesc j);
    hipError_t launch(hipStream_t st, bool with_amax = false);
    PackBatch() = default;
    PackBatch(const PackBatch &) = delete;
    PackBatch &operator=(const PackBatch &) = delete;
    ~PackBatch();
};
struct FoldJobDesc {
    const float *g, *b, *rm, *rv;
    float eps;
    int C;
    float *scale, *shift;
};
struct FoldBatch {
    std::vector<FoldJobDesc> jobs;
    FoldJobDesc *dev = nullptr;
    bool uploaded = false;
    int maxC = 0;
    void clear();
    void add(const FoldJobDesc &j);
    hipError_t launch(hipStream_t st);
    FoldBatch() = default;
    FoldBatch(const FoldBatch &) = delete;
    FoldBatch &operator=(const FoldBatch &) = delete;
    ~FoldBatch();
};

struct OptTensor { float *p, *g, *m, *v, *vmax; int cls; };
struct OptChunk { int tensor, begin, count; };
struct AdamHyper { float decay, beta1, one_minus_beta1, beta2, one_minus_beta2, sqrt_bc2, eps, step_size; };
constexpr int OPT_MAX_CLASSES = 16;
struct AdamTable { AdamHyper hp[OPT_MAX_CLASSES]; unsigned amsgrad, maximize;  };
hipError_t launch_clip_adamw(const OptTensor *tab, const OptChunk *chunks, int nchunks, float *partial, float *normcoef,
                             float max_norm, const AdamHyper &hp, hipStream_t st);
hipError_t launch_grad_norm(const OptTensor *tab, const OptChunk *chunks, int nchunks, float *partial, float *normcoef,
                            float max_norm, double norm_type, hipStream_t st);
hipError_t launch_adamw_classes(const OptTensor *tab, const OptChunk *chunks, int nchunks, const float *normcoef,
                                const AdamTable &tb, hipStream_t st);
hipError_t launch_grad_scale(const OptTensor *tab, const OptChunk *chunks, int nchunks, const float *normcoef, hipStream_t st);
int opt_partial_floats();

int chan_reduce_blocks(int B, int rows_per_img);
hipError_t launch_chan_reduce(const float *y, const float *dz, const float *z, const float *shift, int B, int rows_per_img,
                              int C, int mode, int relu, float *partial, int Cstride, hipStream_t st, const float *fa = nullptr,
                              const float *fb = nullptr);
hipError_t launch_bn_finalize(const float *partial, int nb, int Cstride, double n, int C, const float *shift,
                              const float *gamma, const float *beta, float eps, float momentum, float *rm, float *rv,
                              long long *nbt, float *a, float *b, float *mean, float *rstd, hipStream_t st,
                              double *fold = nullptr, const unsigned *ymax = nullptr, unsigned *zmax = nullptr, int zrelu = 1);
size_t partial_fold_doubles(int nb, int C);
hipError_t launch_affine_act(const float *y, const float *a, const float *b, const float *res, int B, size_t rows_per_img,
                             int C, int per_sample, int relu, float *z, hipStream_t st, unsigned *amax = nullptr,
                             const float *res_a = nullptr, const float *res_b = nullptr, int res_relu = 0,
                             unsigned *zbits = nullptr);
hipError_t launch_bn_bwd_finalize(const float *partial, int nb, int Cstride, double n, int C, const float *gamma,
                                  const float *mean, const float *rstd, float *dgamma, float *dbeta, float *coef,
                                  hipStream_t st, double *fold = nullptr);
// ... 109 lines not shown
```

### monocon-pytorch_amd/hipmonocon/engine.py

```python
import ctypes as C

import numpy as np
import torch

from . import lib as _lib
from . import netspec

PRED_KEYS = tuple(k for k, _ in netspec.PRED_KEYS)
PRED_CH = tuple(c for _, c in netspec.PRED_KEYS)


def _stream():
    return C.c_void_p(torch.cuda.current_stream().cuda_stream)


def _ptr(t):
    return C.c_void_p(t.data_ptr()) if t is not None else C.c_void_p(0)


def _need_cuda(t, what):
    if not (torch.is_tensor(t) and t.is_cuda):
        raise _lib.MonoconHipError("%s must be a CUDA(HIP) tensor; libmonocon_hip has no CPU path" % what)
    if not t.is_contiguous():
        raise _lib.MonoconHipError("%s must be contiguous" % what)
# ... 381 lines not shown
        return buf.raw

    def comm_init(self, rank, world, unique_id):
        assert len(unique_id) == 128
        with torch.cuda.device(self.device):
            _lib.check(self.h, self.lib.mc_comm_init(self.h, int(rank), int(world), C.c_char_p(unique_id)), "mc_comm_init")
        self.comm_world = int(world)

    def comm_destroy(self):
        _lib.check(self.h, self.lib.mc_comm_destroy(self.h), "mc_comm_destroy")
        self.comm_world = 0

    def comm_set_overlap(self, on):
        _lib.check(self.h, self.lib.mc_comm_set_overlap(self.h, int(bool(on))), "mc_comm_set_overlap")

    def comm_info(self):
        r, w, o, n = C.c_int(0), C.c_int(0), C.c_int(0), C.c_int(0)
        la = C.c_ulonglong(0)
        path = C.create_string_buffer(256)
        _lib.check(self.h, self.lib.mc_comm_info(self.h, C.byref(r), C.byref(w), C.byref(o), C.byref(n), C.byref(la), path, 256),
                   "mc_comm_info")
        return {"rank": r.value, "world": w.value, "overlap": bool(o.value), "collectives_per_exchange": n.value,
                "launches": la.value, "library": path.value.decode()}

    def comm_exposed_ms(self):
        ms = C.c_float(-1.0)
        _lib.check(self.h, self.lib.mc_comm_exposed_ms(self.h, C.byref(ms)), "mc_comm_exposed_ms")
        return float(ms.value)

    def allreduce_grads(self):
        with torch.cuda.device(self.device):
            _lib.check(self.h, self.lib.mc_allreduce_grads(self.h, _stream()), "mc_allreduce_grads")

    def build_train_plan(self, B, H, W):
        with torch.cuda.device(self.device):
            _lib.check(self.h, self.lib.mc_build_train_plan(self.h, int(B), int(H), int(W)), "mc_build_train_plan")

    def tune_export(self):
        n = C.c_int(0)
        _lib.check(self.h, self.lib.mc_tune_export(self.h, None, 0, C.byref(n)), "mc_tune_export")
        buf = (C.c_int * max(n.value, 1))()
        _lib.check(self.h, self.lib.mc_tune_export(self.h, buf, n.value, C.byref(n)), "mc_tune_export")
        return list(buf[:n.value])

    def tune_import(self, table):
        buf = (C.c_int * max(len(table), 1))(*[int(v) for v in table])
        rc = self.lib.mc_tune_import(self.h, buf, len(table))
        if rc < 0:
            _lib.check(self.h, rc, "mc_tune_import")
        return rc

    def set_conv_cfg(self, cfg):
        _lib.check(self.h, self.lib.mc_set_conv_cfg(self.h, int(cfg)), "mc_set_conv_cfg")

    def op_conv(self, srcs, weight, stride=1, scale=None, bias=None, residual=None, relu=False):
        for s in srcs:
            _need_cuda(s, "src")
        B, H, W, _ = srcs[0].shape
        Cout, _, k, _ = weight.shape
        Ho = (H + 2 * (k // 2) - k) // stride + 1
        Wo = (W + 2 * (k // 2) - k) // stride + 1
        out = torch.empty((B, Ho, Wo, Cout), dtype=torch.float32, device=srcs[0].device)
        sp = (C.c_void_p * len(srcs))(*[s.data_ptr() for s in srcs])
        sc = (C.c_int * len(srcs))(*[s.shape[3] for s in srcs])
        with torch.cuda.device(out.device):
            rc = self.lib.mc_op_conv(self.h, sp, sc, len(srcs), B, H, W, _ptr(_need_cuda(weight, "weight")), Cout, k,
                                     stride, _ptr(scale), _ptr(bias), _ptr(residual), int(relu), _ptr(out), _stream())
        _lib.check(self.h, rc, "mc_op_conv")
        return out

    def op_conv_dgrad(self, dy, weight, in_hw, c_off=0, cs=None, stride=1, accumulate_into=None):
        _need_cuda(dy, "dy"); _need_cuda(weight, "weight")
        B, Ho, Wo, Cout = dy.shape
        _, cin_total, k, _ = weight.shape
        cs = cin_total - c_off if cs is None else cs
        Hin, Win = in_hw
        out = accumulate_into if accumulate_into is not None else torch.empty((B, Hin, Win, cs), dtype=torch.float32, device=dy.device)
        with torch.cuda.device(dy.device):
            rc = self.lib.mc_op_conv_dgrad(self.h, _ptr(dy), _ptr(weight), B, Hin, Win, cin_total, c_off, cs, Cout, k, stride,
                                           int(accumulate_into is not None), _ptr(out), _stream())
        _lib.check(self.h, rc, "mc_op_conv_dgrad")
        return out

    def op_conv_wgrad(self, srcs, dy, ksize, stride=1):
        B, H, W, _ = srcs[0].shape
        Cout = dy.shape[3]
        cin = sum(s.shape[3] for s in srcs)
        dw = torch.empty((Cout, cin, ksize, ksize), dtype=torch.float32, device=dy.device)
        sp = (C.c_void_p * len(srcs))(*[_need_cuda(s, "src").data_ptr() for s in srcs])
        sc = (C.c_int * len(srcs))(*[s.shape[3] for s in srcs])
        with torch.cuda.device(dy.device):
            rc = self.lib.mc_op_conv_wgrad(self.h, sp, sc, len(srcs), B, H, W, _ptr(_need_cuda(dy, "dy")), Cout, ksize,
                                           stride, _ptr(dw), _stream())
        _lib.check(self.h, rc, "mc_op_conv_wgrad")
        return dw

    def op_stem(self, img, weight, scale, bias):
        B, _, H, W = img.shape
        out = torch.empty((B, H, W, 16), dtype=torch.float32, device=img.device)
        with torch.cuda.device(out.device):
            rc = self.lib.mc_op_stem(self.h, _ptr(_need_cuda(img, "img")), B, H, W, _ptr(weight), _ptr(scale),
                                     _ptr(bias), _ptr(out), _stream())
        _lib.check(self.h, rc, "mc_op_stem")
        return out

    def op_maxpool2(self, x):
        B, H, W, Cc = x.shape
        out = torch.empty((B, H // 2, W // 2, Cc), dtype=torch.float32, device=x.device)
        with torch.cuda.device(out.device):
            rc = self.lib.mc_op_maxpool2(self.h, _ptr(_need_cuda(x, "x")), B, H, W, Cc, _ptr(out), _stream())
        _lib.check(self.h, rc, "mc_op_maxpool2")
        return out

    def op_deconv4x4(self, x, weight):
        B, H, W, Cc = x.shape
        out = torch.empty((B, 2 * H, 2 * W, Cc), dtype=torch.float32, device=x.device)
        with torch.cuda.device(out.device):
            rc = self.lib.mc_op_deconv4x4(self.h, _ptr(_need_cuda(x, "x")), B, H, W, Cc, _ptr(weight), _ptr(out),
                                          _stream())
        _lib.check(self.h, rc, "mc_op_deconv4x4")
        return out

    def to_nhwc(self, x):
        B, Cc, H, W = x.shape
        out = torch.empty((B, H, W, Cc), dtype=torch.float32, device=x.device)
        with torch.cuda.device(out.device):
            rc = self.lib.mc_op_nchw_to_nhwc(self.h, _ptr(_need_cuda(x, "x")), B, Cc, H, W, _ptr(out), _stream())
        _lib.check(self.h, rc, "mc_op_nchw_to_nhwc")
        return out

    def to_nchw(self, x):
        B, H, W, Cc = x.shape
        out = torch.empty((B, Cc, H, W), dtype=torch.float32, device=x.device)
        with torch.cuda.device(out.device):
            rc = self.lib.mc_op_nhwc_to_nchw(self.h, _ptr(_need_cuda(x, "x")), B, Cc, H, W, _ptr(out), _stream())
        _lib.check(self.h, rc, "mc_op_nhwc_to_nchw")
        return out


def p2_inverse(P2):
    P2 = np.asarray(P2, dtype=np.float64).reshape(-1, 3, 4)
    out = np.zeros((P2.shape[0], 4, 4), dtype=np.float64)
    for i, p in enumerate(P2):
        v = np.eye(4)
        v[:3, :4] = p
        out[i] = np.linalg.inv(v)
    return out.astype(np.float32)
```

### monocon-pytorch_amd/hipmonocon/lib.py

```python
import ctypes as C
import os

_HERE = os.path.dirname(os.path.abspath(__file__))
LIB_PATH = os.path.join(_HERE, "libmonocon_hip.so")

MC_F32, MC_I64 = 0, 1
NUM_PREDS = 10

EXPORTS = (
    "mc_create", "mc_destroy", "mc_last_error", "mc_version", "mc_bind_params", "mc_pack_params",
    "mc_forward_infer", "mc_backbone_forward", "mc_neck_forward", "mc_head_forward", "mc_decode", "mc_make_targets", "mc_losses", "mc_losses_backward", "mc_losses_backward_pred", "mc_forward_train", "mc_backward", "mc_backward_pred_grads", "mc_backward_image_grad", "mc_train_generation", "mc_head_forward_train", "mc_head_backward", "mc_head_backward_pred_grads", "mc_train_debug_node", "mc_infer_debug_node", "mc_optim_bind", "mc_clip_adamw_step", "mc_optim_bind_classes", "mc_clip_adamw_step_classes", "mc_clip_bind", "mc_clip_grad_norm", "mc_op_conv", "mc_op_conv_wgrad", "mc_op_conv_dgrad", "mc_op_stem", "mc_op_stem_dgrad", "mc_op_stem_dgrad_fused", "mc_op_maxpool2", "mc_op_deconv4x4",
    "mc_op_nchw_to_nhwc", "mc_op_nhwc_to_nchw", "mc_workspace_bytes", "mc_query_workspace", "mc_forward_cost",
    "mc_preprocess", "mc_preprocess_augmented", "mc_profile_forward", "mc_profile_train", "mc_set_precision", "mc_set_local_maximum_kernel", "mc_set_conv_cfg", "mc_bench_conv", "mc_bench_mfma_peak",
    "mc_comm_unique_id", "mc_comm_init", "mc_comm_destroy", "mc_comm_set_overlap", "mc_comm_info", "mc_comm_exposed_ms", "mc_allreduce_grads",
    "mc_build_train_plan", "mc_tune_export", "mc_tune_import",
    "mc_rotate_iou_eval", "mc_box3d_overlap", "mc_kitti_image_overlap", "mc_kitti_statistics_part",
    "mc_kitti_format", "mc_nms3d",
)


class TensorDesc(C.Structure):
    _fields_ = [("name", C.c_char_p), ("ptr", C.c_void_p), ("numel", C.c_int64), ("dtype", C.c_int32)]


class Labels(C.Structure):
    _fields_ = [(n, C.c_void_p) for n in ("gt_bboxes", "gt_labels", "gt_bboxes_3d", "depths", "gt_kpts_2d",
                                          "gt_kpts_valid_mask", "mask")]


TARGET_FIELDS = ("center_heatmap_target", "wh_target", "offset_target", "dim_target", "alpha_cls_target",
                 "alpha_offset_target", "depth_target", "center2kpt_offset_target", "kpt_heatmap_target",
                 "kpt_heatmap_offset_target", "indices", "indices_kpt", "mask_target", "mask_center2kpt_offset",
                 "mask_kpt_heatmap_offset")


class Targets(C.Structure):
    _fields_ = [(n, C.c_void_p) for n in TARGET_FIELDS]


OPT_MAX_CLASSES = 16


class OptimClass(C.Structure):
    _fields_ = [(n, C.c_double) for n in ("lr", "beta1", "beta2", "eps", "weight_decay")] + \
               [(n, C.c_int) for n in ("step", "amsgrad", "maximize")]


class MonoconHipError(RuntimeError):
    pass


_lib = None


def load():
    global _lib
    if _lib is not None:
        return _lib
    if not os.path.exists(LIB_PATH):
        raise MonoconHipError(
            "libmonocon_hip.so not found at %s -- build it with `python -c 'import __graft_entry__ as g; "
            "g.build()'` or `make -C monocon-pytorch_amd/csrc`; there is no CPU fallback." % LIB_PATH)
    import torch
    lib = C.CDLL(LIB_PATH)
    vp, i, f = C.c_void_p, C.c_int, C.c_float
    fp = C.POINTER(C.c_float)
    lib.mc_version.restype = i
    lib.mc_create.argtypes = [i, C.POINTER(vp)]
    lib.mc_destroy.argtypes = [vp]
    lib.mc_last_error.argtypes = [vp]
    lib.mc_last_error.restype = C.c_char_p
    lib.mc_bind_params.argtypes = [vp, C.POINTER(TensorDesc), i]
    lib.mc_pack_params.argtypes = [vp, i, vp]
    lib.mc_forward_infer.argtypes = [vp, vp, i, i, i, C.POINTER(vp), vp, vp]
    lib.mc_backbone_forward.argtypes = [vp, vp, i, i, i, C.POINTER(vp), vp]
    lib.mc_neck_forward.argtypes = [vp, C.POINTER(vp), i, i, i, vp, vp]
    lib.mc_head_forward.argtypes = [vp, vp, i, i, i, C.POINTER(vp), vp]
    lib.mc_decode.argtypes = [vp, C.POINTER(vp), vp, vp, i, i, i, i, i, f, f, f, vp, vp, vp, vp, vp, vp, vp, vp]
    lib.mc_make_targets.argtypes = [vp, C.POINTER(Labels), i, i, i, i, i, i, C.POINTER(Targets), vp]
    lib.mc_losses.argtypes = [vp, C.POINTER(vp), C.POINTER(Targets), i, i, i, i, vp, vp]
    lib.mc_losses_backward.argtypes = [vp, C.POINTER(vp), C.POINTER(Targets), i, i, i, i, vp, C.POINTER(vp), vp]
    lib.mc_losses_backward_pred.argtypes = lib.mc_losses_backward.argtypes
    lib.mc_forward_train.argtypes = [vp, vp, C.POINTER(Labels), i, i, i, i, C.POINTER(vp), vp, vp]
    lib.mc_backward.argtypes = [vp, vp, vp]
    lib.mc_backward_pred_grads.argtypes = [vp, vp, C.POINTER(vp), vp]
    lib.mc_backward_image_grad.argtypes = [vp, vp, C.POINTER(vp), vp, vp]
    lib.mc_head_forward_train.argtypes = [vp, vp, C.POINTER(Labels), i, i, i, i, C.POINTER(vp), vp, vp]
    lib.mc_head_backward.argtypes = [vp, vp, vp, vp]
    lib.mc_head_backward_pred_grads.argtypes = [vp, vp, C.POINTER(vp), vp, vp]
    lib.mc_train_generation.argtypes = [vp, C.POINTER(C.c_ulonglong)]
    lib.mc_train_debug_node.argtypes = [vp, i, i, vp, C.POINTER(i), vp]
    lib.mc_infer_debug_node.argtypes = [vp, i, i, vp, C.POINTER(i), vp]
    d = C.c_double
    lib.mc_optim_bind.argtypes = [vp, i, C.POINTER(vp), C.POINTER(vp), C.POINTER(vp), C.POINTER(vp), C.POINTER(C.c_int64)]
    lib.mc_clip_adamw_step.argtypes = [vp, d, d, d, d, d, d, i, vp, vp]
    lib.mc_optim_bind_classes.argtypes = [vp, i, C.POINTER(vp), C.POINTER(vp), C.POINTER(vp), C.POINTER(vp), C.POINTER(vp),
                                          C.POINTER(C.c_int64), C.POINTER(i)]
    lib.mc_clip_adamw_step_classes.argtypes = [vp, C.POINTER(OptimClass), i, d, d, vp, vp]
    lib.mc_clip_bind.argtypes = [vp, i, C.POINTER(vp), C.POINTER(C.c_int64)]
    lib.mc_clip_grad_norm.argtypes = [vp, d, d, vp, vp]
    lib.mc_op_conv.argtypes = [vp, C.POINTER(vp), C.POINTER(i), i, i, i, i, vp, i, i, i, vp, vp, vp, i, vp, vp]
    lib.mc_op_conv_wgrad.argtypes = [vp, C.POINTER(vp), C.POINTER(i), i, i, i, i, vp, i, i, i, vp, vp]
    lib.mc_op_stem.argtypes = [vp, vp, i, i, i, vp, vp, vp, vp, vp]
    lib.mc_op_stem_dgrad.argtypes = [vp, vp, vp, i, i, i, vp, vp]
    lib.mc_op_stem_dgrad_fused.argtypes = [vp, vp, vp, vp, vp, i, i, i, vp, vp]
    lib.mc_op_maxpool2.argtypes = [vp, vp, i, i, i, i, vp, vp]
    lib.mc_op_deconv4x4.argtypes = [vp, vp, i, i, i, i, vp, vp, vp]
    lib.mc_op_nchw_to_nhwc.argtypes = [vp, vp, i, i, i, i, vp, vp]
    lib.mc_op_nhwc_to_nchw.argtypes = [vp, vp, i, i, i, i, vp, vp]
    lib.mc_workspace_bytes.argtypes = [vp]
    lib.mc_query_workspace.argtypes = [vp, i, i, i, i, C.POINTER(C.c_size_t)]
    lib.mc_workspace_bytes.restype = C.c_size_t
    lib.mc_forward_cost.argtypes = [vp, i, i, i, C.POINTER(C.c_double), C.POINTER(C.c_double)]
    lib.mc_profile_forward.argtypes = [vp, i, fp, C.POINTER(i), vp]
    lib.mc_bench_mfma_peak.argtypes = [vp, i, i, fp]
    lib.mc_profile_train.argtypes = [vp, i, C.POINTER(C.c_double), C.POINTER(C.c_double), C.POINTER(C.c_double), C.POINTER(i), vp]
    lib.mc_preprocess.argtypes = [vp, vp, i, i, i, C.POINTER(C.c_double), C.POINTER(C.c_double), i, i, vp, vp]
    lib.mc_preprocess_augmented.argtypes = [vp, vp, vp, i, i, i, C.POINTER(C.c_double), C.POINTER(C.c_double), i, i, vp, vp]
    lib.mc_op_conv_dgrad.argtypes = [vp, vp, vp, i, i, i, i, i, i, i, i, i, i, vp, vp]
    lib.mc_comm_unique_id.argtypes = [vp, vp]
    lib.mc_comm_init.argtypes = [vp, i, i, vp]
    lib.mc_comm_destroy.argtypes = [vp]
    lib.mc_comm_set_overlap.argtypes = [vp, i]
    lib.mc_comm_info.argtypes = [vp, C.POINTER(i), C.POINTER(i), C.POINTER(i), C.POINTER(i), C.POINTER(C.c_ulonglong), C.c_char_p, i]
    lib.mc_comm_exposed_ms.argtypes = [vp, fp]
    lib.mc_allreduce_grads.argtypes = [vp, vp]
    lib.mc_build_train_plan.argtypes = [vp, i, i, i]
    lib.mc_tune_export.argtypes = [vp, C.POINTER(i), i, C.POINTER(i)]
    lib.mc_tune_import.argtypes = [vp, C.POINTER(i), i]
    ll, dp, llp = C.c_longlong, C.POINTER(C.c_double), C.POINTER(C.c_longlong)
    lib.mc_rotate_iou_eval.argtypes = [vp, vp, vp, ll, ll, i, vp, vp]
    lib.mc_box3d_overlap.argtypes = [vp, vp, vp, ll, ll, i, vp, vp]
    lib.mc_kitti_image_overlap.argtypes = [dp, ll, dp, ll, i, dp]
    lib.mc_kitti_statistics_part.argtypes = [i, dp, ll, llp, llp, llp, dp, dp, dp, llp, llp, i, C.c_double, dp, ll, i, dp, dp, llp]
    lib.mc_kitti_format.argtypes = [vp, vp, vp, vp, vp, vp, vp, i, i, vp, vp, vp, vp, vp]
    lib.mc_nms3d.argtypes = [vp, vp, vp, vp, vp, i, i, i, f, i, vp, vp, vp]
    lib.mc_set_precision.argtypes = [vp, i]
    lib.mc_set_local_maximum_kernel.argtypes = [vp, i]
    lib.mc_set_conv_cfg.argtypes = [vp, i]
    lib.mc_bench_conv.argtypes = [vp, i, i, i, i, C.POINTER(i), i, i, i, i, i, fp]
    for name in EXPORTS:
        fn = getattr(lib, name)
        if fn.restype is C.c_int or name not in ("mc_last_error", "mc_workspace_bytes"):
            if name not in ("mc_last_error", "mc_workspace_bytes"):
                fn.restype = i
    _lib = lib
    return lib


def check(handle, rc, what):
    if rc != 0:
        msg = load().mc_last_error(handle)
        raise MonoconHipError("%s failed (rc=%d): %s" % (what, rc, msg.decode() if msg else "?"))
```

Baseline: 683.3 images/sec.

## Merge per-source data-gradient convolutions into one multi-destination launch

Adds a multi-destination mode to the fp16/bf16 MFMA conv kernel. A stride-1 conv whose input was a concatenation of several sources can now compute all source data gradients in a single launch: the weights are packed into one panel with per-destination column offsets, and each wave picks its destination's epilogue (output pointer, accumulate flag, BM fused epilogue). This removes the repeated reads of dy and the extra launches of the old per-source dgrad loop. The new path is enabled by default in the train plan through a switch and autotuned per shape. In exchange it adds runtime epilogue branching, column padding per destination, and possibly a less ideal tile choice.

```diff
diff --git a/include/monocon_hip.h b/include/monocon_hip.h
--- a/include/monocon_hip.h
+++ b/include/monocon_hip.h
@@ -138,6 +138,8 @@
                     const float *weight, float *out, void *stream);
 int mc_op_conv_dgrad(mc_handle *h, const float *dy, const float *weight_oihw, int B, int Hin, int Win, int CinTotal,
                      int c_off, int Cs, int Cout, int ksize, int stride, int accumulate, float *dx, void *stream);
+int mc_op_conv_dgrad_multi(mc_handle *h, const float *dy, const float *weight_oihw, int B, int H, int W, int Cout, int ksize,
+                           int nsrc, const int src_channels[], float *const dx[], unsigned accumulate_mask, void *stream);
 int mc_op_nchw_to_nhwc(mc_handle *h, const float *in, int B, int C, int H, int W, float *out,
                        void *stream);
 int mc_op_nhwc_to_nchw(mc_handle *h, const float *in, int B, int C, int H, int W, float *out,
diff --git a/monocon-pytorch_amd/csrc/conv_bf16.hip b/monocon-pytorch_amd/csrc/conv_bf16.hip
--- a/monocon-pytorch_amd/csrc/conv_bf16.hip
+++ b/monocon-pytorch_amd/csrc/conv_bf16.hip
@@ -29,9 +29,10 @@
     static constexpr size_t LDS_BYTES = TILE_BYTES + PB * 16;
 };
 
-template <int KS, int S, int WM, int WN, int WTM, int WTN, int SPL, bool BM = false, bool LZ = false>
+template <int KS, int S, int WM, int WN, int WTM, int WTN, int SPL, bool BM = false, bool LZ = false, bool MD = false>
 __global__ __launch_bounds__(64 * WM * WN, SPL == 1 ? 3 : 2) void conv_bf16_kernel(const ConvArgs a) {
     static_assert(!LZ || (SPL == 2 && !BM), "lazy sources: forward launches of the fp16-split mode");
+    static_assert(!MD || (!BM && !LZ && S == 1 && (KS == 3 || KS == 1)), "multi-destination: stride-1 data gradients; BM is chosen per destination");
     using Cfg = ConvCfgB16<KS, S, WM, WN, WTM, WTN, SPL>;
     typedef typename Piece<SPL>::T pc_t;
     typedef typename Piece<SPL>::V8 pc8;
@@ -150,7 +151,27 @@
     pc8 bq[DB][SPL][WTN];
 #pragma unroll
     for (int j = 0; j < DB - 1; ++j) load_b(bq[j], 0, j);
-    const EpiCoef<WTN> coef = conv_epi_coef<WN, WTN, BM>(a, n0, wn, li);
+    [[maybe_unused]] ConvArgs ae_md;
+    const ConvArgs &ae = [&]() -> const ConvArgs & { if constexpr (MD) return ae_md; else return a; }();
+    int n0e = n0;
+    if constexpr (MD) {
+        ConvArgs &ae = ae_md;
+        ae = a;
+        const int ncol = n0 + wn * WTN * 32;
+        int dj = 0;
+#pragma unroll
+        for (int j = 1; j < 4; ++j) dj = (j < a.ndst && ncol >= a.dst[j].col0) ? j : dj;
+        const ConvDst &d = a.dst[dj];
+        n0e = n0 - d.col0;
+        ae.Cout = d.C; ae.CoutP = d.CP;
+        ae.out = d.out; ae.out_ld = d.out_ld; ae.out_coff = 0;
+        ae.o_px = d.out_ld; ae.o_row = a.Wout * d.out_ld; ae.o_img = a.Hout * a.Wout * d.out_ld;
+        ae.res = d.accumulate ? d.out : nullptr; ae.res_ld = d.out_ld;
+        ae.r_px = ae.o_px; ae.r_row = ae.o_row; ae.r_img = ae.o_img;
+        ae.bm_y = d.bm_y; ae.bm_z = d.bm_z; ae.bm_zbits = d.bm_zbits; ae.bm_a = d.bm_a; ae.bm_b = d.bm_b; ae.bm_relu = d.bm_relu;
+        ae.stats = d.stats; ae.amax_out = d.amax_out;
+    }
+    const EpiCoef<WTN> coef = conv_epi_coef<WN, WTN, BM || MD>(ae, n0e, wn, li);
 
 #ifndef MC_CONV_PF
 #define MC_CONV_PF 1
@@ -329,7 +350,12 @@
 #pragma unroll
                 for (int r = 0; r < 16; ++r) acc[tm][tn][r] += accm[tm][tn][r];
     }
-    conv_epilogue<WM, WN, WTM, WTN, BNT, BM>(a, acc, pinfo, chunk * PB, img, n0, wm, wn, g, li, coef, omul);
+    if constexpr (MD) {
+        if (ae.bm_y) conv_epilogue<WM, WN, WTM, WTN, BNT, true>(ae, acc, pinfo, chunk * PB, img, n0e, wm, wn, g, li, coef, omul);
+        else conv_epilogue<WM, WN, WTM, WTN, BNT, false>(ae, acc, pinfo, chunk * PB, img, n0e, wm, wn, g, li, coef, omul);
+    } else {
+        conv_epilogue<WM, WN, WTM, WTN, BNT, BM>(ae, acc, pinfo, chunk * PB, img, n0e, wm, wn, g, li, coef, omul);
+    }
 #ifdef MC_PHASE_TIMERS
     if (a.phase_prof && lane == 0) {
         __builtin_amdgcn_s_waitcnt(0);
@@ -345,6 +371,19 @@
 static hipError_t launch_b16_one(ConvArgs a, hipStream_t st, ConvArgs *resolved) {
     using Cfg = ConvCfgB16<KS, S, Sh::WM, Sh::WN, Sh::WTM, Sh::WTN, SPL>;
     static_assert(Cfg::PB == Sh::PB && Cfg::BNT == Sh::BNT, "the shape table and the kernel agree on the tile");
+    if constexpr (!BM && !LZ) {
+        if (a.ndst > 1) {
+            if constexpr (S == 1 && (KS == 3 || KS == 1)) {
+                if (a.ndst > 4 || conv_any_lazy(a) || a.CoutP % Cfg::BNT || !conv_dst_span_ok(a, Sh::WTN * 32)) return hipErrorInvalidValue;
+                conv_set_patches(a, Cfg::PB);
+                if (resolved) *resolved = a;
+                return launch_dyn_lds<conv_bf16_kernel<KS, S, Sh::WM, Sh::WN, Sh::WTM, Sh::WTN, SPL, false, false, true>>(
+                    Cfg::LDS_BYTES, dim3((unsigned)(a.B * a.chunks * (a.CoutP / Cfg::BNT))), dim3(Cfg::NT), st, a);
+            } else {
+                return hipErrorInvalidValue;
+            }
+        }
+    }
     if constexpr (!LZ) {
         if (conv_any_lazy(a)) {
             if constexpr (SPL == 2 && !BM && (KS == 3 || KS == 1)) {
diff --git a/monocon-pytorch_amd/csrc/conv_mfma.h b/monocon-pytorch_amd/csrc/conv_mfma.h
--- a/monocon-pytorch_amd/csrc/conv_mfma.h
+++ b/monocon-pytorch_amd/csrc/conv_mfma.h
@@ -30,6 +30,18 @@
 __device__ __forceinline__ float lazy_act(float y, float a, float b, float cap) {
     return __builtin_amdgcn_fmed3f(__builtin_fmaf(y, a, b), 0.f, cap);
 }
+
+struct ConvDst {
+    float *out;
+    int out_ld, accumulate;
+    int col0, C, CP;
+    const float *bm_y, *bm_z;
+    const unsigned *bm_zbits;
+    const float *bm_a, *bm_b;
+    int bm_relu;
+    float *stats;
+    unsigned *amax_out;
+};
 
 struct ConvArgs {
     ConvSrc src[4];
@@ -62,7 +74,18 @@
     const unsigned *amax_w;
     unsigned *amax_out;
     unsigned long long *phase_prof;
-};
+    int ndst;
+    ConvDst dst[4];
+};
+inline bool conv_dst_span_ok(const ConvArgs &a, int span) {
+    int end = 0;
+    for (int j = 0; j < a.ndst; ++j) {
+        const ConvDst &d = a.dst[j];
+        if (d.col0 % span || d.col0 < end || d.C < 1) return false;
+        end = d.col0 + d.C;
+    }
+    return end <= a.CoutP;
+}
 
 __host__ __device__ __forceinline__ int f16_scale_exp(unsigned amax_bits) {
     const int E = (int)((amax_bits >> 23) & 0xffu);
@@ -434,6 +457,8 @@
                                 int accumulate, const unsigned *amax_dy, const unsigned *amax_w, hipStream_t st);
 
 hipError_t launch_conv(const ConvArgs &a, int ks, int stride, hipStream_t st, ConvArgs *resolved = nullptr);
+bool conv_multi_dst_ok(const ConvArgs &a, int ks, int stride);
+int conv_pick_cfg_multi(const ConvArgs &a, int ks, int stride);
 bool conv_lazy_capable(const ConvArgs &a, int ks, int stride);
 
 struct ProfLast { int kind; double flops, bytes; };
diff --git a/monocon-pytorch_amd/csrc/conv_mfma.hip b/monocon-pytorch_amd/csrc/conv_mfma.hip
--- a/monocon-pytorch_amd/csrc/conv_mfma.hip
+++ b/monocon-pytorch_amd/csrc/conv_mfma.hip
@@ -362,6 +362,17 @@
     return conv_bf16_ok(a, ks, stride) && (ks == 3 || ks == 1);
 }
 
+int conv_pick_cfg_multi(const ConvArgs &a, int ks, int stride) {
+    const int c = conv_pick_cfg(a.Cout, a.CoutP, ks, stride, a.B, a.Hout, a.Wout);
+    const ConvShape s = conv_shape(c);
+    if (conv_dst_span_ok(a, s.WTN * 32)) return c;
+    return s.BNT() == 128 ? CFG_64x128 : (s.BNT() == 64 ? CFG_64x64 : CFG_128x32);
+}
+
+bool conv_multi_dst_ok(const ConvArgs &a, int ks, int stride) {
+    return a.ndst > 1 && a.ndst <= 4 && stride == 1 && (ks == 3 || ks == 1) && a.prec >= 1 && !conv_any_lazy(a) && conv_bf16_ok(a, ks, stride);
+}
+
 hipError_t launch_conv(const ConvArgs &a_in, int ks, int stride, hipStream_t st, ConvArgs *resolved) {
     ConvArgs a = a_in;
     const bool lazy = conv_any_lazy(a);
@@ -369,6 +380,13 @@
     if (dense_out) { a.o_px = a.out_ld; a.o_row = a.Wout * a.out_ld; a.o_img = a.Hout * a.Wout * a.out_ld; }
     if (a.r_px == 0) { a.r_px = a.res_ld; a.r_row = a.Wout * a.res_ld; a.r_img = a.Hout * a.Wout * a.res_ld; }
     if (a.cfg == CFG_SMALL && !dense_out) return hipErrorInvalidValue;
+    if (a.ndst > 1) {
+        if (!conv_multi_dst_ok(a, ks, stride) || (a.cfg & ~(CFG_SHAPE_BITS | CFG_WRES))) return hipErrorInvalidValue;
+        a.cfg &= CFG_SHAPE_BITS;
+        if (a.cfg == CFG_AUTO) a.cfg = conv_pick_cfg_multi(a, ks, stride);
+        prof_last = conv_cost(a, ks);
+        return launch_conv_bf16(a, ks, stride, st, resolved);
+    }
     int sc[4];
     for (int i = 0; i < a.nsrc; ++i) sc[i] = a.src[i].C;
     const int ck = conv_ck(ks, stride, sc, a.nsrc);
diff --git a/monocon-pytorch_amd/csrc/mc_api.hip b/monocon-pytorch_amd/csrc/mc_api.hip
--- a/monocon-pytorch_amd/csrc/mc_api.hip
+++ b/monocon-pytorch_amd/csrc/mc_api.hip
@@ -302,6 +302,41 @@
 }
 
 int mc_choose_conv_cfg(mc_handle *h, const ConvArgs &a_in, int ks, int stride) {
+    if (a_in.ndst > 1) {
+        if (h->force_cfg) return h->force_cfg;
+        const int heuristic = conv_pick_cfg_multi(a_in, ks, stride);
+        if (h->dry_alloc || !h->autotune) return heuristic;
+        std::vector<int> key = {a_in.B, a_in.Hin, a_in.Win, ks, stride, a_in.Cout, a_in.CoutP, a_in.nsrc, 2 * a_in.prec | 128 | (a_in.ndst << 8)};
+        for (int i = 0; i < a_in.nsrc; ++i) key.push_back(a_in.src[i].C);
+        for (int j = 0; j < a_in.ndst; ++j) key.push_back(a_in.dst[j].C | (a_in.dst[j].accumulate ? 1 << 16 : 0));
+        auto it = h->tuned.find(key);
+        if (it != h->tuned.end()) return it->second;
+        hipEvent_t e0, e1;
+        if (hipEventCreate(&e0) != hipSuccess || hipEventCreate(&e1) != hipSuccess) return heuristic;
+        ConvArgs a = a_in;
+        int best = heuristic;
+        float best_ms = 1e30f;
+        for (const ConvShape &s : CONV_SHAPES) {
+            if (a.CoutP % s.BNT() || !conv_dst_span_ok(a, s.WTN * 32)) continue;
+            a.cfg = s.id;
+            if (launch_conv(a, ks, stride, nullptr) != hipSuccess) { (void)hipGetLastError(); continue; }
+            float t_min = 1e30f;
+            for (int rep = 0; rep < 3; ++rep) {
+                (void)hipEventRecord(e0, nullptr);
+                (void)launch_conv(a, ks, stride, nullptr);
+                (void)hipEventRecord(e1, nullptr);
+                if (hipEventSynchronize(e1) != hipSuccess) { t_min = 1e30f; break; }
+                float ms = 0.f;
+                (void)hipEventElapsedTime(&ms, e0, e1);
+                t_min = std::min(t_min, ms);
+            }
+            if (t_min < best_ms) { best_ms = t_min; best = s.id; }
+        }
+        (void)hipEventDestroy(e0);
+        (void)hipEventDestroy(e1);
+        h->tuned[key] = best;
+        return best;
+    }
     const bool small_ok = conv_small_ok(a_in, ks, stride);
     if (h->dry_alloc)
         return (small_ok && !(a_in.prec >= 1 && conv_bf16_ok(a_in, ks, stride))) ? (int)CFG_SMALL
diff --git a/monocon-pytorch_amd/csrc/mc_train_api.hip b/monocon-pytorch_amd/csrc/mc_train_api.hip
--- a/monocon-pytorch_amd/csrc/mc_train_api.hip
+++ b/monocon-pytorch_amd/csrc/mc_train_api.hip
@@ -236,6 +236,68 @@
         const int kk = mc::dgrad_conv_args(d, pack.jobs[c], h->prec, dy, dy_amax, B, Ho, Wo, Cout, dx, Hin, Win, accumulate != 0);
         d.cfg = h->force_cfg;
         e = mc::launch_conv(d, kk, 1, st);
+    }
+    hipError_t e2 = hipStreamSynchronize(st);
+    HIPCHK(h, e);
+    HIPCHK(h, e2);
+    return 0;
+}
+
+int mc_op_conv_dgrad_multi(mc_handle *h, const float *dy, const float *weight_oihw, int B, int H, int W, int Cout, int ksize, int nsrc,
+                           const int src_channels[], float *const dx[], unsigned accumulate_mask, void *stream) {
+    if (!h) return -1;
+    if (!dy || !weight_oihw || !dx || !src_channels || nsrc < 1 || nsrc > 4) return fail(h, "mc_op_conv_dgrad_multi: bad argument");
+    if (ksize != 3 && ksize != 1) return fail(h, "mc_op_conv_dgrad_multi: unsupported k=%d (stride 1 only)", ksize);
+    int CinTotal = 0;
+    for (int j = 0; j < nsrc; ++j) {
+        if (!dx[j] || src_channels[j] < 4 || src_channels[j] % 4) return fail(h, "mc_op_conv_dgrad_multi: source %d: null / C %% 4", j);
+        CinTotal += src_channels[j];
+    }
+    if (Cout % 16) return fail(h, "mc_op_conv_dgrad_multi: Cout must be a multiple of 16");
+    HIPCHK(h, hipSetDevice(h->device));
+    hipStream_t st = static_cast<hipStream_t>(stream);
+    const mc::DgradMulti L = mc::dgrad_multi_layout(src_channels, nsrc);
+    bool merged = nsrc > 1 && h->prec >= 1 && mc::panel_has_pieces(h->prec, Cout) && Cout % 32 == 0;
+    if (merged && h->force_cfg) merged = mc::dgrad_multi_cfg_fits(h->force_cfg, L);
+    if (!merged) {
+        int c_off = 0;
+        for (int j = 0; j < nsrc; ++j) {
+            const int rc = mc_op_conv_dgrad(h, dy, weight_oihw, B, H, W, CinTotal, c_off, src_channels[j], Cout, ksize, 1,
+                                            (accumulate_mask >> j) & 1u, dx[j], stream);
+            if (rc) return rc;
+            c_off += src_channels[j];
+        }
+        return 0;
+    }
+    ScratchBuf slots;
+    unsigned *dy_amax = nullptr, *w_amax = nullptr;
+    if (h->prec == 3) {
+        const size_t ndy = (size_t)B * H * W * Cout;
+        HIPCHK(h, op_amax_slots(slots, &dy, &ndy, 1, weight_oihw, (size_t)Cout * CinTotal * ksize * ksize, true, st));
+        dy_amax = slots.as<unsigned>();
+        w_amax = dy_amax + 4 * mc::AMAX_WORDS;
+    }
+    const size_t pn = mc::dgrad_multi_panel_elems(ksize, Cout, L), bytes16 = pn * 2 * mc::split_pieces(h->prec);
+    ScratchBuf panel, panel16;
+    HIPCHK(h, panel.alloc(pn * 4));
+    HIPCHK(h, hipMemsetAsync(panel.p, 0, pn * 4, st));
+    HIPCHK(h, panel16.alloc(bytes16));
+    HIPCHK(h, hipMemsetAsync(panel16.p, 0, bytes16, st));
+    mc::PackBatch pack;
+    bool acc[4];
+    int c_off = 0;
+    for (int j = 0; j < nsrc; ++j) {
+        pack.add(mc::pack_job_dgrad(weight_oihw, Cout, CinTotal, ksize, c_off, src_channels[j], Cout, -1, panel.as<float>(), panel16.p,
+                                    h->prec, w_amax, L.col0[j], L.CsP));
+        c_off += src_channels[j];
+        acc[j] = ((accumulate_mask >> j) & 1u) != 0;
+    }
+    hipError_t e = pack.launch(st);
+    if (e == hipSuccess) {
+        mc::ConvArgs d;
+        mc::dgrad_multi_conv_args(d, L, ksize, Cout, panel.as<float>(), panel16.p, w_amax, h->prec, dy, dy_amax, B, H, W, Cout, dx, acc);
+        d.cfg = h->force_cfg;
+        e = mc::launch_conv(d, ksize, 1, st);
     }
     hipError_t e2 = hipStreamSynchronize(st);
     HIPCHK(h, e);
diff --git a/monocon-pytorch_amd/csrc/mc_train_plan.hip b/monocon-pytorch_amd/csrc/mc_train_plan.hip
--- a/monocon-pytorch_amd/csrc/mc_train_plan.hip
+++ b/monocon-pytorch_amd/csrc/mc_train_plan.hip
@@ -20,6 +20,7 @@
     long long head_dx_fuse;
     long long head_zskip;
     long long dgrad_s2_thin;
+    long long dgrad_merge;
     long long stem_fuse;
     long long bm_epilogue;
     long long wres_bwd;
@@ -37,6 +38,7 @@
     {"MONOCON_HIP_HEAD_DX_FUSE", &PlanSwitches::head_dx_fuse, 1},
     {"MONOCON_HIP_HEAD_ZSKIP", &PlanSwitches::head_zskip, 1},
     {"MONOCON_HIP_DGRAD_S2_THIN", &PlanSwitches::dgrad_s2_thin, 1},
+    {"MONOCON_HIP_DGRAD_MERGE", &PlanSwitches::dgrad_merge, 1},
     {"MONOCON_HIP_STEM_FUSE", &PlanSwitches::stem_fuse, 1},
     {"MONOCON_HIP_BM_EPILOGUE", &PlanSwitches::bm_epilogue, 1},
     {"MONOCON_HIP_WRES_BWD", &PlanSwitches::wres_bwd, 0},
@@ -72,8 +74,9 @@
         PoolBwdArgs *pool;
         float **deconv_stats;
     };
+    int dst = -1;
     LastWriter() : conv(nullptr) {}
-    LastWriter(ConvArgs *c) : kind(c ? DGRAD_CONV : NONE), conv(c) {}
+    LastWriter(ConvArgs *c, int dst_ = -1) : kind(c ? DGRAD_CONV : NONE), conv(c), dst(dst_) {}
     LastWriter(PoolBwdArgs *p) : kind(p ? POOL_BWD : NONE), pool(p) {}
     LastWriter(float **s) : kind(s ? DECONV_BWD : NONE), deconv_stats(s) {}
 };
@@ -488,6 +491,49 @@
         wrote(srcnode, (d.cfg == CFG_SMALL && !conv_thin_ok(d, ks, 1)) ? nullptr : dp);
     }
 
+    bool emit_dgrad_merged(const float *w_master, const Tensor &dy, const Rec &r) {
+        const int ks = r.L->ks, n = (int)r.srcs.size(), Cout_fwd = r.L->cout;
+        if (!sw.dgrad_merge || !ts->ok || r.L->stride != 1 || (ks != 3 && ks != 1) || n < 2 || n > 4) return false;
+        if (h->prec < 1 || !panel_has_pieces(h->prec, Cout_fwd) || dy.C % 32 || (h->prec == 3 && (!dy.amax || !w_slot(w_master)))) return false;
+        int Cs[4];
+        for (int j = 0; j < n; ++j) {
+            const TNode &sn = ts->nodes[r.srcs[j]];
+            if (!sn.needs_grad || sn.t.H != dy.H || sn.t.W != dy.W) return false;
+            for (int i = 0; i < j; ++i)
+                if (r.srcs[i] == r.srcs[j]) return false;
+            Cs[j] = sn.t.C;
+        }
+        const DgradMulti L = dgrad_multi_layout(Cs, n);
+        auto fits = [&](int cfg) { return dgrad_multi_cfg_fits(cfg, L); };
+        if (h->force_cfg && !fits(h->force_cfg)) return false;
+        float *g[4];
+        bool acc[4];
+        for (int j = 0; j < n; ++j) { g[j] = g_acquire(r.srcs[j]); acc[j] = ts->nodes[r.srcs[j]].ginit; }
+        const size_t pn = dgrad_multi_panel_elems(ks, Cout_fwd, L);
+        float *dst = alloc(pn);
+        void *dst16 = alloc((3 * pn + 1) / 2);
+        ConvArgs d;
+        dgrad_multi_conv_args(d, L, ks, Cout_fwd, dst, dst16, w_slot(w_master), h->prec, dy.p, dy.amax, dy.B, dy.H, dy.W, dy.C, g, acc);
+        if (!conv_multi_dst_ok(d, ks, 1)) return false;
+        d.cfg = mc_choose_conv_cfg(h, d, ks, 1);
+        if (!fits(d.cfg)) return false;
+        d.cfg &= CFG_SHAPE_BITS;
+        int c_off = 0;
+        for (int j = 0; j < n; ++j) {
+            ts->pack_batch.add(pack_job_dgrad(w_master, Cout_fwd, r.L->cin, ks, c_off, Cs[j], Cout_fwd, -1, dst, dst16, h->prec,
+                                              w_slot(w_master), L.col0[j], L.CsP));
+            c_off += Cs[j];
+        }
+        ts->dgrads.push_back(d);
+        ConvArgs *dp = &ts->dgrads.back();
+        push_bwd([=](mc_handle *hh, hipStream_t st) { HIPCHK(hh, launch_conv(*dp, ks, 1, st)); return 0; });
+        for (int j = 0; j < n; ++j) wrote(r.srcs[j], LastWriter(dp, j));
+        if (sw.plan_debug)
+            fprintf(stderr, "[plan] merged dgrad %-36s k %d  cfg %3d  K %4d  %d destinations, %d columns (%d owned)  %dx%d\n", r.L->conv.c_str(),
+                    ks, d.cfg, d.Cin, n, d.CoutP, c_off, d.Hout, d.Wout);
+        return true;
+    }
+
     int emit_wgrad(const std::vector<int> &srcs, const Tensor &dy, int dy_ld, int Cout, int ks, int stride, float *dw) {
         WgradArgs a{};
         const std::vector<const Tensor *> xs = conv_sources(srcs);
@@ -541,18 +587,29 @@
         if (sw.plan_debug)
             fprintf(stderr, "[plan] bn_backward %-40s %4d ch %4dx%-4d relu %d res %d last-writer-conv %d\n", bn.c_str(), C, r.y.H,
                     r.y.W, relu, r.res >= 0, lc != nullptr);
-        if (lc && lc->out == zn.g && lc->Cout == C && lc->out_ld == C && lc->Hout == r.y.H && lc->Wout == r.y.W && !lc->stats) {
-            const int ppi = conv_chunks_per_image(lc->cfg, r.y.H, r.y.W), nbp = B * ppi, cstride = lc->CoutP;
+        ConvDst *ld = (lc && last.dst >= 0) ? &lc->dst[last.dst] : nullptr;
+        const bool lc_fits = lc && lc->Hout == r.y.H && lc->Wout == r.y.W &&
+                             (ld ? (ld->out == zn.g && ld->C == C && ld->out_ld == C && !ld->stats)
+                                 : (lc->out == zn.g && lc->Cout == C && lc->out_ld == C && !lc->stats));
+        if (lc_fits) {
+            const int ppi = conv_chunks_per_image(lc->cfg, r.y.H, r.y.W), nbp = B * ppi, cstride = ld ? ld->CP : lc->CoutP;
             float *partial = alloc((size_t)nbp * cstride * 2);
-            lc->stats = partial;
-            lc->bm_y = yp; lc->bm_z = zp; lc->bm_a = fa; lc->bm_b = fb; lc->bm_relu = relu;
-            lc->bm_zbits = relu == 1 ? r.zbits : nullptr;
-            if (sw.wres_bwd >= 1 && !(lc->cfg & (CFG_SMALL | CFG_WS)) && conv_wres_ok(*lc, 3, 1)) lc->cfg |= CFG_WRES;
+            if (ld) {
+                ld->stats = partial;
+                ld->bm_y = yp; ld->bm_z = zp; ld->bm_a = fa; ld->bm_b = fb; ld->bm_relu = relu;
+                ld->bm_zbits = relu == 1 ? r.zbits : nullptr;
+            } else {
+                lc->stats = partial;
+                lc->bm_y = yp; lc->bm_z = zp; lc->bm_a = fa; lc->bm_b = fb; lc->bm_relu = relu;
+                lc->bm_zbits = relu == 1 ? r.zbits : nullptr;
+                if (sw.wres_bwd >= 1 && !(lc->cfg & (CFG_SMALL | CFG_WS)) && conv_wres_ok(*lc, 3, 1)) lc->cfg |= CFG_WRES;
+            }
             if (sw.plan_debug)
                 fprintf(stderr, "[plan]   twin of %-36s cfg %3d  K %4d  Cout %3d  %dx%d  res %d  nsrc %d srcC %d wres %d\n", bn.c_str(), lc->cfg,
-                        lc->Cin, lc->Cout, lc->Hout, lc->Wout, lc->res != nullptr, lc->nsrc, lc->src[0].C, (lc->cfg & CFG_WRES) != 0);
+                        lc->Cin, C, lc->Hout, lc->Wout, ld ? ld->accumulate : lc->res != nullptr, lc->nsrc, lc->src[0].C,
+                        (lc->cfg & CFG_WRES) != 0);
             const bool skip_affine = caller_forms_dy && !gres;
-            if (skip_affine) lc->amax_out = dymax;
+            if (skip_affine) (ld ? ld->amax_out : lc->amax_out) = dymax;
             return step(partial, nbp, cstride, false, !skip_affine);
         }
         PoolBwdArgs *pl = last.kind == LastWriter::POOL_BWD ? last.pool : nullptr;
@@ -782,10 +839,12 @@
         const int64_t wn = (int64_t)r.L->cout * r.L->cin * r.L->ks * r.L->ks;
         const int wgrad = emit_wgrad(r.srcs, dy, r.L->cout, r.L->cout, r.L->ks, r.L->stride, G(r.L->conv + ".weight", wn));
         const float *wm = P(r.L->conv + ".weight", wn);
-        int c_off = 0;
-        for (int s : r.srcs) {
-            emit_dgrad(wm, dy, r.L->cout, r.L->cin, r.L->ks, r.L->stride, c_off, s, r.L->cout);
-            c_off += ts->nodes[s].t.C;
+        if (!emit_dgrad_merged(wm, dy, r)) {
+            int c_off = 0;
+            for (int s : r.srcs) {
+                emit_dgrad(wm, dy, r.L->cout, r.L->cin, r.L->ks, r.L->stride, c_off, s, r.L->cout);
+                c_off += ts->nodes[s].t.C;
+            }
         }
         g_release(r.z, wgrad);
     }
diff --git a/monocon-pytorch_amd/csrc/pack_batch.hip b/monocon-pytorch_amd/csrc/pack_batch.hip
--- a/monocon-pytorch_amd/csrc/pack_batch.hip
+++ b/monocon-pytorch_amd/csrc/pack_batch.hip
@@ -173,8 +173,9 @@
                         float v[8];
 #pragma unroll
                         for (int q = 0; q < 8; ++q) v[q] = src[(size_t)q * j.CinTotal * KK + tap];
-                        const size_t i32a = (((size_t)tapd * (j.CoutP >> 2) + n8 * 2) * j.CsP + cl) * 4;
-                        put8(v, i32a, i32a + (size_t)j.CsP * 4, (((size_t)tapd * (j.CoutP >> 3) + n8) * j.CsP + cl) * 8, plane);
+                        const int col = cl + j.n_off;
+                        const size_t i32a = (((size_t)tapd * (j.CoutP >> 2) + n8 * 2) * j.CsP + col) * 4;
+                        put8(v, i32a, i32a + (size_t)j.CsP * 4, (((size_t)tapd * (j.CoutP >> 3) + n8) * j.CsP + col) * 8, plane);
                     }
                 }
             };
@@ -195,9 +196,10 @@
                 tapd = dr * (1 + px) + ds;
             }
             float rem = j.w[(((size_t)n * j.CinTotal + j.c_off + cl) * k + r) * k + s];
-            if (j.dst32) j.dst32[(((size_t)tapd * (j.CoutP >> 2) + (n >> 2)) * j.CsP + cl) * 4 + (n & 3)] = rem;
+            const int col = cl + j.n_off;
+            if (j.dst32) j.dst32[(((size_t)tapd * (j.CoutP >> 2) + (n >> 2)) * j.CsP + col) * 4 + (n & 3)] = rem;
             if (d16)
-                store_pieces_b(rem * wscale, d16 + (((size_t)tapd * (j.CoutP >> 3) + (n >> 3)) * j.CsP + cl) * 8 + (n & 7), plane,
+                store_pieces_b(rem * wscale, d16 + (((size_t)tapd * (j.CoutP >> 3) + (n >> 3)) * j.CsP + col) * 8 + (n & 7), plane,
                                j.nsplit);
         }
     }
diff --git a/monocon-pytorch_amd/csrc/train.h b/monocon-pytorch_amd/csrc/train.h
--- a/monocon-pytorch_amd/csrc/train.h
+++ b/monocon-pytorch_amd/csrc/train.h
@@ -69,12 +69,50 @@
     return j;
 }
 inline PackJobDesc pack_job_dgrad(const float *w, int Cout, int CinTotal, int k, int c_off, int Cs, int CoutPad, int cls,
-                                  float *dst32, void *dst16, int prec, unsigned *amax) {
+                                  float *dst32, void *dst16, int prec, unsigned *amax, int n_off = 0, int CsP = 0) {
     PackJobDesc j{};
     j.w = w; j.dst32 = dst32; j.dst16 = panel_has_pieces(prec, CoutPad) ? dst16 : nullptr;
     j.kind = 1; j.Cout = Cout; j.Cin = Cs; j.k = k; j.CinTotal = CinTotal; j.CoutP = CoutPad; j.c_off = c_off;
-    j.CsP = conv_coutp(Cs); j.cls = cls; j.nsplit = split_pieces(prec); j.amax = amax;
+    j.n_off = n_off;
+    j.CsP = CsP ? CsP : conv_coutp(Cs); j.cls = cls; j.nsplit = split_pieces(prec); j.amax = amax;
     return j;
+}
+struct DgradMulti {
+    int n, col0[4], C[4], CsP;
+};
+inline DgradMulti dgrad_multi_layout(const int *Cs, int n) {
+    DgradMulti L{};
+    L.n = n;
+    int col = 0;
+    for (int j = 0; j < n && j < 4; ++j) { L.col0[j] = col; L.C[j] = Cs[j]; col += conv_coutp(Cs[j]); }
+    L.CsP = conv_coutp(col);
+    return L;
+}
+inline bool dgrad_multi_cfg_fits(int cfg, const DgradMulti &L) {
+    const ConvShape s = conv_shape(cfg);
+    if (!s.id || (cfg & ~(CFG_SHAPE_BITS | CFG_WRES)) || L.CsP % s.BNT()) return false;
+    for (int j = 0; j < L.n; ++j)
+        if (L.col0[j] % (s.WTN * 32)) return false;
+    return true;
+}
+inline size_t dgrad_multi_panel_elems(int k, int CoutPad, const DgradMulti &L) { return (size_t)k * k * CoutPad * L.CsP; }
+inline void dgrad_multi_conv_args(ConvArgs &d, const DgradMulti &L, int k, int CoutPad, float *dst32, void *dst16, unsigned *w_amax,
+                                  int prec, const float *dy, const unsigned *dy_amax, int B, int Hd, int Wd, int Cd, float *const g[],
+                                  const bool accumulate[]) {
+    (void)k;
+    d = ConvArgs{};
+    d.nsrc = 1; d.src[0].p = dy; d.src[0].C = Cd;
+    d.B = B; d.Hin = Hd; d.Win = Wd; d.Hout = Hd; d.Wout = Wd;
+    d.Cin = Cd; d.Cout = L.col0[L.n - 1] + L.C[L.n - 1]; d.CoutP = L.CsP; d.wpk = dst32;
+    d.wpk16 = panel_has_pieces(prec, CoutPad) ? dst16 : nullptr; d.prec = d.wpk16 ? prec : 0;
+    d.amax_in[0] = dy_amax; d.amax_w = w_amax;
+    d.ndst = L.n;
+    for (int j = 0; j < L.n; ++j) {
+        ConvDst &t = d.dst[j];
+        t.out = g[j]; t.out_ld = L.C[j]; t.accumulate = accumulate[j] ? 1 : 0;
+        t.col0 = L.col0[j]; t.C = L.C[j]; t.CP = conv_coutp(L.C[j]);
+    }
+    d.out = g[0]; d.out_ld = L.C[0];
 }
 inline int dgrad_conv_args(ConvArgs &d, const PackJobDesc &p, int prec, const float *dy, const unsigned *dy_amax, int B, int Hd,
                            int Wd, int Cd, float *g, int Hs, int Ws, bool accumulate) {
diff --git a/monocon-pytorch_amd/hipmonocon/engine.py b/monocon-pytorch_amd/hipmonocon/engine.py
--- a/monocon-pytorch_amd/hipmonocon/engine.py
+++ b/monocon-pytorch_amd/hipmonocon/engine.py
@@ -487,6 +487,22 @@
         _lib.check(self.h, rc, "mc_op_conv_dgrad")
         return out
 
+    def op_conv_dgrad_multi(self, dy, weight, widths, accumulate_into=None):
+        _need_cuda(dy, "dy"); _need_cuda(weight, "weight")
+        B, H, W, Cout = dy.shape
+        _, cin_total, k, _ = weight.shape
+        widths = [int(c) for c in widths]
+        assert sum(widths) == cin_total, (widths, cin_total)
+        acc = list(accumulate_into) if accumulate_into is not None else [None] * len(widths)
+        outs = [a if a is not None else torch.empty((B, H, W, c), dtype=torch.float32, device=dy.device) for a, c in zip(acc, widths)]
+        mask = sum(1 << j for j, a in enumerate(acc) if a is not None)
+        wc = (C.c_int * len(widths))(*widths)
+        op = (C.c_void_p * len(widths))(*[_need_cuda(o, "dx").data_ptr() for o in outs])
+        with torch.cuda.device(dy.device):
+            rc = self.lib.mc_op_conv_dgrad_multi(self.h, _ptr(dy), _ptr(weight), B, H, W, Cout, k, len(widths), wc, op, mask, _stream())
+        _lib.check(self.h, rc, "mc_op_conv_dgrad_multi")
+        return outs
+
     def op_conv_wgrad(self, srcs, dy, ksize, stride=1):
         B, H, W, _ = srcs[0].shape
         Cout = dy.shape[3]
diff --git a/monocon-pytorch_amd/hipmonocon/lib.py b/monocon-pytorch_amd/hipmonocon/lib.py
--- a/monocon-pytorch_amd/hipmonocon/lib.py
+++ b/monocon-pytorch_amd/hipmonocon/lib.py
@@ -9,7 +9,7 @@
 
 EXPORTS = (
     "mc_create", "mc_destroy", "mc_last_error", "mc_version", "mc_bind_params", "mc_pack_params",
-    "mc_forward_infer", "mc_backbone_forward", "mc_neck_forward", "mc_head_forward", "mc_decode", "mc_make_targets", "mc_losses", "mc_losses_backward", "mc_losses_backward_pred", "mc_forward_train", "mc_backward", "mc_backward_pred_grads", "mc_backward_image_grad", "mc_train_generation", "mc_head_forward_train", "mc_head_backward", "mc_head_backward_pred_grads", "mc_train_debug_node", "mc_infer_debug_node", "mc_optim_bind", "mc_clip_adamw_step", "mc_optim_bind_classes", "mc_clip_adamw_step_classes", "mc_clip_bind", "mc_clip_grad_norm", "mc_op_conv", "mc_op_conv_wgrad", "mc_op_conv_dgrad", "mc_op_stem", "mc_op_stem_dgrad", "mc_op_stem_dgrad_fused", "mc_op_maxpool2", "mc_op_deconv4x4",
+    "mc_forward_infer", "mc_backbone_forward", "mc_neck_forward", "mc_head_forward", "mc_decode", "mc_make_targets", "mc_losses", "mc_losses_backward", "mc_losses_backward_pred", "mc_forward_train", "mc_backward", "mc_backward_pred_grads", "mc_backward_image_grad", "mc_train_generation", "mc_head_forward_train", "mc_head_backward", "mc_head_backward_pred_grads", "mc_train_debug_node", "mc_infer_debug_node", "mc_optim_bind", "mc_clip_adamw_step", "mc_optim_bind_classes", "mc_clip_adamw_step_classes", "mc_clip_bind", "mc_clip_grad_norm", "mc_op_conv", "mc_op_conv_wgrad", "mc_op_conv_dgrad", "mc_op_conv_dgrad_multi", "mc_op_stem", "mc_op_stem_dgrad", "mc_op_stem_dgrad_fused", "mc_op_maxpool2", "mc_op_deconv4x4",
     "mc_op_nchw_to_nhwc", "mc_op_nhwc_to_nchw", "mc_workspace_bytes", "mc_query_workspace", "mc_forward_cost",
     "mc_preprocess", "mc_preprocess_augmented", "mc_profile_forward", "mc_profile_train", "mc_set_precision", "mc_set_local_maximum_kernel", "mc_set_conv_cfg", "mc_bench_conv", "mc_bench_mfma_peak",
     "mc_comm_unique_id", "mc_comm_init", "mc_comm_destroy", "mc_comm_set_overlap", "mc_comm_info", "mc_comm_exposed_ms", "mc_allreduce_grads",
@@ -118,6 +118,7 @@
     lib.mc_preprocess.argtypes = [vp, vp, i, i, i, C.POINTER(C.c_double), C.POINTER(C.c_double), i, i, vp, vp]
     lib.mc_preprocess_augmented.argtypes = [vp, vp, vp, i, i, i, C.POINTER(C.c_double), C.POINTER(C.c_double), i, i, vp, vp]
     lib.mc_op_conv_dgrad.argtypes = [vp, vp, vp, i, i, i, i, i, i, i, i, i, i, vp, vp]
+    lib.mc_op_conv_dgrad_multi.argtypes = [vp, vp, vp, i, i, i, i, i, i, C.POINTER(C.c_int), C.POINTER(vp), C.c_uint, vp]
     lib.mc_comm_unique_id.argtypes = [vp, vp]
     lib.mc_comm_init.argtypes = [vp, i, i, vp]
     lib.mc_comm_destroy.argtypes = [vp]
```

After: 687.0 images/sec (median of 6 runs). About the same (+0.5%).
